# nameofuser1/vad

Measured on NVIDIA B200. Metric: audio_seconds_per_second, higher is better.
Workload: dtype f32

## Files before the change

### include/vadb200.h

```cpp
#ifndef VADB200_H_
#define VADB200_H_

#include <stdint.h>

#ifdef __cplusplus
extern "C" {
#endif

#define VADB200_VERSION 201

#define VADB200_OK 0
#define VADB200_E_INVALID (-1)
#define VADB200_E_UNSUPPORTED (-2)
#define VADB200_E_CUDA (-3)
#define VADB200_E_NOMEM (-4)
#define VADB200_E_STATE (-5)

#define VADB200_MODE_MFCC 0
#define VADB200_MODE_DATASET 1
#define VADB200_MODE_VAD 2

#define VADB200_FEAT_ANALYSER 0
#define VADB200_FEAT_DATASET 1

typedef struct vadb200_handle vadb200_handle;
typedef struct vadb200_plan vadb200_plan;
typedef struct vadb200_bank vadb200_bank;
typedef struct vadb200_trainer vadb200_trainer;

typedef struct vadb200_config {
  int32_t sample_rate;
  int32_t frame_size;
  int32_t frame_step;
  int32_t fft_n;
  int32_t n_filters;
  int32_t n_mfcc;
  double low_hz;
  double high_hz;
  int32_t lifter_l;
  int32_t reserved;
} vadb200_config;

const char* vadb200_last_error(void);
int vadb200_version(void);
void vadb200_default_config(vadb200_config* cfg);

int64_t vadb200_frames_for_length(int64_t n_samples);
int64_t vadb200_outputs_for_length(int64_t n_samples);

int vadb200_create(const vadb200_config* cfg, int device, vadb200_handle** out);
int vadb200_destroy(vadb200_handle* h);

int vadb200_get_filterbank(vadb200_handle* h, double* h_out);

int vadb200_set_ffn_weights(vadb200_handle* h, const float* W1, const float* b1, const float* W2,
                            const float* b2, const float* W3, const float* b3, const float* W4,
                            const float* b4);

int vadb200_set_ffn_impl(vadb200_handle* h, int impl);
int vadb200_get_ffn_impl(vadb200_handle* h);

int vadb200_set_frontend(vadb200_handle* h, float preemph, const float* h_window );
int vadb200_get_frontend(vadb200_handle* h, float* preemph, float* h_window , int* has_window);
int vadb200_set_decision_threshold(vadb200_handle* h, float p_voiced);
float vadb200_get_decision_threshold(vadb200_handle* h);

int vadb200_plan_create(vadb200_handle* h, const int64_t* h_offsets, const int64_t* h_lengths,
                        int64_t n_utt, int mode, vadb200_plan** out);
int vadb200_plan_destroy(vadb200_plan* p);
int64_t vadb200_plan_total_rows(const vadb200_plan* p);
int vadb200_plan_row_offsets(const vadb200_plan* p, int64_t* h_out );
int64_t vadb200_plan_segment_frames(const vadb200_plan* p);
int64_t vadb200_plan_segment_count(const vadb200_plan* p);
int vadb200_set_plan_segment_frames(vadb200_handle* h, int frames);

int vadb200_mfcc_packed(vadb200_plan* p, const int16_t* d_pcm, int64_t pcm_len, float* d_out,
                        void* stream);

int vadb200_vad_packed(vadb200_plan* p, const int16_t* d_pcm, int64_t pcm_len, uint8_t* d_labels,
                       float* d_logits, float* d_feats, int feat_mode, void* stream);

int vadb200_vad_host(vadb200_plan* p, const int16_t* h_pcm, int64_t pcm_len, uint8_t* h_labels,
                     float* h_logits , int feat_mode);
int vadb200_set_host_chunk_samples(vadb200_handle* h, int64_t samples);
int vadb200_mfcc_host(vadb200_plan* p, const int16_t* h_pcm, int64_t pcm_len, float* h_out);

int64_t vadb200_plan_max_speech_segments(const vadb200_plan* p);
int64_t vadb200_plan_speech_workspace_bytes(const vadb200_plan* p);
int vadb200_plan_speech_segments(vadb200_plan* p, const uint8_t* d_labels ,
                                 int min_speech_rows, int min_silence_rows, int pad_rows,
                                 uint8_t* d_smoothed ,
                                 int64_t* d_segments ,
                                 int64_t* d_segment_offsets ,
                                 int64_t* d_speech_offsets ,
                                 void* d_workspace, int64_t workspace_bytes, void* stream);
int vadb200_plan_gather_speech(vadb200_plan* p, const int16_t* d_pcm, int64_t pcm_len,
                               const int64_t* d_segments, const int64_t* d_segment_offsets,
                               const int64_t* d_speech_offsets, int16_t* d_out ,
                               int64_t out_capacity, void* stream);

int vadb200_scale_rows(vadb200_handle* h, float* d_rows, int64_t n_rows, double* h_stats, void* stream);
int vadb200_ingest_pcm(vadb200_handle* h, const void* d_raw, int big_endian, const int64_t* d_src_start,
                       const int64_t* d_dst_start, const int64_t* d_len, int n_seg, int64_t max_len,
                       int16_t* d_dst, void* stream);

int vadb200_spec_frames(vadb200_handle* h, const float* d_frames, int64_t n, int frame_len,
                        float* d_spec , void* stream);
int vadb200_mfcc_frames(vadb200_handle* h, const float* d_frames, int64_t n, int frame_len,
                        float* d_mfcc , void* stream);
int vadb200_mfcc_from_spec(vadb200_handle* h, const float* d_spec , int64_t n,
                           float* d_mfcc , void* stream);

int vadb200_vad_windows(vadb200_handle* h, const float* d_windows, int64_t n, int feat_mode,
                        uint8_t* d_labels , float* d_logits ,
                        float* d_feats , void* stream);
int vadb200_ffn_predict(vadb200_handle* h, const float* d_x, int64_t n, uint8_t* d_labels,
                        float* d_logits , void* stream);

int vadb200_get_deltas(vadb200_handle* h, const float* d_a, const float* d_b, int64_t n,
                       float* d_out, void* stream);
int vadb200_lifter(vadb200_handle* h, const float* d_in, int64_t n_rows, int ncoef, int L,
                   float* d_out, void* stream);

int vadb200_stream_bank_create(vadb200_handle* h, int n_streams, vadb200_bank** out);
int vadb200_stream_bank_destroy(vadb200_bank* b);
int vadb200_stream_bank_reset(vadb200_bank* b, void* stream);
int vadb200_stream_feed(vadb200_bank* b, const int16_t* d_chunks ,
                        uint8_t* d_labels , float* d_logits ,
                        void* stream);

int vadb200_trainer_create(vadb200_handle* h, int64_t max_batch, float lr, float rho, float eps,
                           vadb200_trainer** out);
int vadb200_trainer_destroy(vadb200_trainer* t);
int vadb200_trainer_set_weights(vadb200_trainer* t, const float* W1, const float* b1, const float* W2,
                                const float* b2, const float* W3, const float* b3, const float* W4,
                                const float* b4, int reset_optimizer);
int vadb200_trainer_get_weights(vadb200_trainer* t, float* W1, float* b1, float* W2, float* b2, float* W3,
                                float* b3, float* W4, float* b4);
int vadb200_train_on_batch(vadb200_trainer* t, const float* d_x, const uint8_t* d_y, int64_t n,
                           float* h_loss, void* stream);

int vadb200_synth_pcm(vadb200_handle* h, int16_t* d_out, int64_t n_utt, int64_t utt_samples,
                      int64_t utt_stride, uint32_t seed, int64_t first_utt, void* stream);
int vadb200_fp32_peak(vadb200_handle* h, int variant, int iters, double* tflops_out);
int64_t vadb200_launch_count(void);

#ifdef __cplusplus
}
#endif
#endif
```

### vad_b200/_lib.py

```python
import ctypes as C
import os

HERE = os.path.dirname(os.path.abspath(__file__))
LIB_PATH = os.environ.get("VADB200_LIB") or os.path.join(HERE, "libvadb200.so")


class VadB200Error(RuntimeError):
    def __init__(self, code, msg):
        RuntimeError.__init__(self, "vadb200 error %d: %s" % (code, msg))
        self.code = code


class Config(C.Structure):
    _fields_ = [("sample_rate", C.c_int32), ("frame_size", C.c_int32), ("frame_step", C.c_int32),
                ("fft_n", C.c_int32), ("n_filters", C.c_int32), ("n_mfcc", C.c_int32),
                ("low_hz", C.c_double), ("high_hz", C.c_double), ("lifter_l", C.c_int32),
                ("reserved", C.c_int32)]


_P = C.c_void_p
_I64 = C.c_int64
SIGNATURES = {
    "vadb200_last_error": (C.c_char_p, []),
    "vadb200_version": (C.c_int, []),
    "vadb200_default_config": (None, [C.POINTER(Config)]),
    "vadb200_frames_for_length": (_I64, [_I64]),
    "vadb200_outputs_for_length": (_I64, [_I64]),
    "vadb200_create": (C.c_int, [C.POINTER(Config), C.c_int, C.POINTER(_P)]),
    "vadb200_destroy": (C.c_int, [_P]),
    "vadb200_get_filterbank": (C.c_int, [_P, _P]),
    "vadb200_set_ffn_weights": (C.c_int, [_P] + [_P] * 8),
    "vadb200_set_ffn_impl": (C.c_int, [_P, C.c_int]),
    "vadb200_get_ffn_impl": (C.c_int, [_P]),
    "vadb200_set_frontend": (C.c_int, [_P, C.c_float, _P]),
    "vadb200_get_frontend": (C.c_int, [_P, _P, _P, _P]),
    "vadb200_set_decision_threshold": (C.c_int, [_P, C.c_float]),
    "vadb200_get_decision_threshold": (C.c_float, [_P]),
    "vadb200_plan_create": (C.c_int, [_P, _P, _P, _I64, C.c_int, C.POINTER(_P)]),
    "vadb200_plan_destroy": (C.c_int, [_P]),
    "vadb200_plan_total_rows": (_I64, [_P]),
    "vadb200_plan_row_offsets": (C.c_int, [_P, _P]),
    "vadb200_plan_segment_frames": (_I64, [_P]),
    "vadb200_plan_segment_count": (_I64, [_P]),
    "vadb200_set_plan_segment_frames": (C.c_int, [_P, C.c_int]),
    "vadb200_mfcc_host": (C.c_int, [_P, _P, _I64, _P]),
    "vadb200_plan_max_speech_segments": (_I64, [_P]),
    "vadb200_plan_speech_workspace_bytes": (_I64, [_P]),
    "vadb200_plan_speech_segments": (C.c_int, [_P, _P, C.c_int, C.c_int, C.c_int, _P, _P, _P, _P, _P, _I64, _P]),
    "vadb200_plan_gather_speech": (C.c_int, [_P, _P, _I64, _P, _P, _P, _P, _I64, _P]),
    "vadb200_scale_rows": (C.c_int, [_P, _P, _I64, _P, _P]),
    "vadb200_ingest_pcm": (C.c_int, [_P, _P, C.c_int, _P, _P, _P, C.c_int, _I64, _P, _P]),
    "vadb200_mfcc_packed": (C.c_int, [_P, _P, _I64, _P, _P]),
    "vadb200_vad_packed": (C.c_int, [_P, _P, _I64, _P, _P, _P, C.c_int, _P]),
    "vadb200_vad_host": (C.c_int, [_P, _P, _I64, _P, _P, C.c_int]),
    "vadb200_set_host_chunk_samples": (C.c_int, [_P, _I64]),
    "vadb200_spec_frames": (C.c_int, [_P, _P, _I64, C.c_int, _P, _P]),
    "vadb200_mfcc_frames": (C.c_int, [_P, _P, _I64, C.c_int, _P, _P]),
    "vadb200_mfcc_from_spec": (C.c_int, [_P, _P, _I64, _P, _P]),
    "vadb200_vad_windows": (C.c_int, [_P, _P, _I64, C.c_int, _P, _P, _P, _P]),
    "vadb200_ffn_predict": (C.c_int, [_P, _P, _I64, _P, _P, _P]),
    "vadb200_get_deltas": (C.c_int, [_P, _P, _P, _I64, _P, _P]),
    "vadb200_lifter": (C.c_int, [_P, _P, _I64, C.c_int, C.c_int, _P, _P]),
    "vadb200_stream_bank_create": (C.c_int, [_P, C.c_int, C.POINTER(_P)]),
    "vadb200_stream_bank_destroy": (C.c_int, [_P]),
    "vadb200_stream_bank_reset": (C.c_int, [_P, _P]),
    "vadb200_stream_feed": (C.c_int, [_P, _P, _P, _P, _P]),
    "vadb200_trainer_create": (C.c_int, [_P, _I64, C.c_float, C.c_float, C.c_float, C.POINTER(_P)]),
    "vadb200_trainer_destroy": (C.c_int, [_P]),
    "vadb200_trainer_set_weights": (C.c_int, [_P] + [_P] * 8 + [C.c_int]),
    "vadb200_trainer_get_weights": (C.c_int, [_P] + [_P] * 8),
    "vadb200_train_on_batch": (C.c_int, [_P, _P, _P, _I64, _P, _P]),
    "vadb200_synth_pcm": (C.c_int, [_P, _P, _I64, _I64, _I64, C.c_uint32, _I64, _P]),
    "vadb200_fp32_peak": (C.c_int, [_P, C.c_int, C.c_int, C.POINTER(C.c_double)]),
    "vadb200_launch_count": (_I64, []),
}

_lib = None


def load():
    global _lib
    if _lib is not None:
        return _lib
    if not os.path.isfile(LIB_PATH):
        raise ImportError(
            "vad_b200: %s is missing -- build it with `python -m vad_b200.build` "
            "(nvcc, sm_100a).  There is no CPU fallback." % LIB_PATH)
    lib = C.CDLL(LIB_PATH)
    for name, (res, args) in SIGNATURES.items():
        fn = getattr(lib, name)
        fn.restype = res
        fn.argtypes = args
    _lib = lib
    return lib


def check(rc):
    if rc != 0:
        raise VadB200Error(rc, load().vadb200_last_error().decode("utf-8", "replace"))
```

### vad_b200/csrc/vad_kernels.cuh

```cuda
#pragma once

#include <cuda_runtime.h>

#include "vad_core.cuh"
#include "ffn_tc.cuh"

namespace vadb {

constexpr int kThreads = 256;
constexpr int kWarps = 8;
constexpr int kStepFrames = 32;
constexpr int kRing = 288;
constexpr int kPPitch = 34;
constexpr int kStageSamples = (kStepFrames - 1) * kHop + kFrame;
constexpr int kStagePad = 5376;
constexpr int kBlockSteps = 8;

constexpr int kOffPcm = 0;
constexpr int kOffExch = kOffPcm + 2 * kStagePad * 2;
constexpr int kOffP = kOffExch + kWarps * 2 * kExchFrame * 8;
constexpr int kP2Bytes = (kP2RowsAlloc * kP2Pitch * 4 + 15) & ~15;
constexpr int kOffLogE = kOffP + kP2Bytes;
constexpr int kLogEFloats = kNMel * 32;
constexpr int kOffRing = kOffLogE + 2 * kLogEFloats * 4;
constexpr int kOffTw1 = kOffRing + ((kRingRows * ring_pitch(kRing) * 4 + 15) & ~15);
constexpr int kOffTw2 = kOffTw1 + 256 * 8;
constexpr int kOffBar = kOffTw2 + 128 * 8;
constexpr int kOffSeg = kOffBar + 48;
constexpr int kFusedSmemBytes = kOffSeg + 16;
constexpr int kBlockStepsTc = 4;
static_assert(kTcBlobBytes <= kWarps * 2 * kExchFrame * 8 + kP2Bytes, "weight blob must fit exch + P");
static_assert(kBlockSteps * kStepFrames * kNFeat * 4 + 16 <= kWarps * 2 * kExchFrame * 8 + kP2Bytes,
              "dataset-row staging tile must fit exch + P");
static_assert(2 * (kFusedSmemBytes + 1024) <= 233472, "two CTAs per SM");

struct Segment {
  long long pcm_start;
  long long out_start;
  int n_frames;
  int cont;
};

struct FrontEnd {
  const cf2* win;
  float preemph;
};

#if defined(VADB_DEBUG_HOOKS)
#define VADB_DBG(p) ((p).debug_skip)
#else
#define VADB_DBG(p) 0
#endif

struct FusedParams {
  const int16_t* pcm;
  long long pcm_len;
  const Segment* segs;
  int seg_begin, seg_end;
  int* counter;
  const cf2* tw1;
  const cf2* tw2;
  uint8_t* labels;
  float* logits;
  float* feats;
  float* rows;
  long long row_base;
  int feat_mode;
  const unsigned char* tc_blob;
  long long* dbg_ts;
  int debug_skip;
};

__device__ __forceinline__ uint32_t smem_u32(const void* p) {
  return static_cast<uint32_t>(__cvta_generic_to_shared(p));
}
__device__ __forceinline__ void mbar_init(uint64_t* bar, uint32_t count) {
  asm volatile("mbarrier.init.shared::cta.b64 [%0], %1;" ::"r"(smem_u32(bar)), "r"(count) : "memory");
}
__device__ __forceinline__ void fence_mbar_init() {
  asm volatile("fence.mbarrier_init.release.cluster;" ::: "memory");
}
__device__ __forceinline__ void mbar_arrive_expect_tx(uint64_t* bar, uint32_t bytes) {
  asm volatile("mbarrier.arrive.expect_tx.shared::cta.b64 _, [%0], %1;" ::"r"(smem_u32(bar)), "r"(bytes)
               : "memory");
}
__device__ __forceinline__ void mbar_arrive(uint64_t* bar) {
  asm volatile("mbarrier.arrive.shared::cta.b64 _, [%0];" ::"r"(smem_u32(bar)) : "memory");
}
__device__ __forceinline__ void warp_arrive(uint64_t* bar, int lane) {
  __syncwarp();
  if (lane == 0) mbar_arrive(bar);
}
__device__ __forceinline__ bool mbar_try_wait(uint64_t* bar, uint32_t parity) {
  uint32_t ok;
  asm volatile(
      "{\n\t.reg .pred p;\n\t"
      "mbarrier.try_wait.parity.shared::cta.b64 p, [%1], %2;\n\t"
      "selp.u32 %0, 1, 0, p;\n\t}"
      : "=r"(ok)
      : "r"(smem_u32(bar)), "r"(parity)
      : "memory");
  return ok != 0;
}
__device__ __forceinline__ void mbar_wait(uint64_t* bar, uint32_t parity) {
  while (!mbar_try_wait(bar, parity)) {
  }
}
__device__ __forceinline__ void bulk_g2s(void* dst_smem, const void* src_gmem, uint32_t bytes, uint64_t* bar) {
  asm volatile(
      "cp.async.bulk.shared::cluster.global.mbarrier::complete_tx::bytes [%0], [%1], %2, [%3];" ::"r"(
          smem_u32(dst_smem)),
      "l"(src_gmem), "r"(bytes), "r"(smem_u32(bar))
      : "memory");
}

struct ShflXchg {
  int lane;
  __device__ __forceinline__ float operator()(float mine, int, bool, int partner) const {
    return __shfl_sync(0xffffffffu, mine, (lane & 16) | partner);
  }
  __device__ __forceinline__ f2 operator()(f2 mine, int, bool, int partner) const {
    const int src = (lane & 16) | partner;
    return mk2(__shfl_sync(0xffffffffu, mine.x, src), __shfl_sync(0xffffffffu, mine.y, src));
  }
};

template <int NZ, class LOAD, class PRE, class STORE>
__device__ __forceinline__ void warp_fft_quad(LOAD&& load, f2* ex, const cf2* s_tw1, const cf2* s_tw2, int lane,
                                               PRE&& before_store, STORE&& store) {
  const int t = lane & 15;
  f2 xr[16], xi[16];
  load(t, xr, xi);
  fft_pass1<NZ>(xr, xi, s_tw1, t);
  exch_store_plane(ex, t, xr);
  __syncwarp();
  exch_load_plane(ex, t, xr);
  __syncwarp();
  exch_store_plane(ex, t, xi);
  __syncwarp();
  exch_load_plane(ex, t, xi);
  __syncwarp();
  dft16<16>(xr, xi);
  before_store();
  fft_split_store(xr, xi, t, s_tw2, ShflXchg{lane}, store);
}
struct P2Store {
  static constexpr bool kHasSink = true;
  float* lo_base;
  float* hi_base;
  float* lo0;
  float* mid_ptr;
  __device__ __forceinline__ P2Store(float* P2, int col, int k1) {
    lo_base = P2 + p2_index(k1, col);
    hi_base = P2 + p2_index(256 - k1, col);
    float* sink = P2 + kP2Rows * kP2Pitch + k1 + 2 * (col & 8);
    lo0 = k1 >= kMelFirstBin ? lo_base : sink;
    mid_ptr = k1 == 0 ? P2 + p2_index(128, col) : sink;
  }
  static __device__ __forceinline__ void put(float* q, f2 v) {
    q[0] = v.x;
    q[2] = v.y;
  }
  template <class K> __device__ __forceinline__ void lo(K, f2 v) const {
    constexpr int k2 = K::value;
    if constexpr (k2 == 0) put(lo0, v);
    else put(lo_base + 8 * k2 * kP2Pitch, v);
  }
  template <class K> __device__ __forceinline__ void hi(K, f2 v) const { put(hi_base - 8 * K::value * kP2Pitch, v); }
  __device__ __forceinline__ void mid(f2 v) const { put(mid_ptr, v); }
};

template <int NZ, class LOAD>
__device__ __forceinline__ void warp_fft_pair(LOAD&& load, cf2* ex, const cf2* s_tw1, const cf2* s_tw2,
                                               float* s_P, int fi, int lane) {
  const int t = lane & 15;
  float xr[16], xi[16];
  load(xr, xi);
  fft_pass1<NZ>(xr, xi, s_tw1, t);
  exch_store(ex, t, xr, xi);
  __syncwarp();
  exch_load(ex, t, xr, xi);
  __syncwarp();
  dft16<16>(xr, xi);
  fft_split_store(xr, xi, t, s_tw2, ShflXchg{lane}, [&](int bin, float v) { s_P[bin * kPPitch + fi] = v; });
}

template <int NTHREADS = kThreads, class GEN>
__device__ __forceinline__ void flush_flat(float* dst, int total, int tid, GEN&& gen) {
  if (total <= 0) return;
  const int head = min(total, static_cast<int>((16u - (reinterpret_cast<uintptr_t>(dst) & 15u)) & 15u) >> 2);
  const int nq = (total - head) >> 2;
  for (int q = tid; q < nq; q += NTHREADS) {
    float v[4];
    gen(head + 4 * q, v, 4);
    *reinterpret_cast<float4*>(dst + head + 4 * q) = make_float4(v[0], v[1], v[2], v[3]);
  }
  const int tail0 = head + 4 * nq;
  if (tid < 2) {
    const int j0 = tid == 0 ? 0 : tail0, cnt = tid == 0 ? head : total - tail0;
    if (cnt > 0) {
      float v[4];
      gen(j0, v, cnt);
#pragma unroll
      for (int i = 0; i < 4; ++i)
        if (i < cnt) dst[j0 + i] = v[i];
    }
  }
}

__device__ __forceinline__ void classify_row(const FfnParams& w, const float (&r)[5][kNCep], int feat_mode,
                                             uint8_t* labels, float* logits, float* feats, long long row, float th) {
  float x[kNFeat];
  const bool ok = window_features(r, feat_mode, x);
  float logit[kNCls];
  ffn_forward(w, x, logit);
  uint8_t lab = decide(logit, th);
  if (!ok) {
    logit[0] = logit[1] = logit[2] = NAN;
    lab = 0;
  }
  if (labels) labels[row] = lab;
  if (logits) {
    logits[row * 3 + 0] = logit[0];
    logits[row * 3 + 1] = logit[1];
    logits[row * 3 + 2] = logit[2];
  }
  if (feats) {
#pragma unroll
    for (int i = 0; i < kNFeat; ++i) feats[row * kNFeat + i] = x[i];
  }
}

template <int MODE, int TC> struct FfnArgOf { using type = FfnNone; };
template <> struct FfnArgOf<2, 0> { using type = FfnParams; };
template <> struct FfnArgOf<2, 1> { using type = FfnBias; };
template <> struct FfnArgOf<2, 2> { using type = FfnBias; };

template <bool FE, class A>
__device__ __forceinline__ uint8_t decide_of(const float (&logit)[kNCls], const A& ffn) {
  if constexpr (FE && !std::is_same<A, FfnNone>::value) return decide(logit, ffn.thresh);
  else return decide(logit);
}

constexpr int kStageOffFe = 8;
static_assert(kStageSamples + kStageOffFe <= kStagePad, "front-end stage offset must fit the PCM buffer");

template <int MODE, int TC, bool FE>
__device__ __forceinline__ void fused_body(const FusedParams& p, const typename FfnArgOf<MODE, TC>::type& ffn,
                                           const FrontEnd& fe, const int tid) {
  static_assert(TC == 0 || MODE == 2, "tensor-core FFN only exists in VAD mode");
  constexpr int kBlk = TC ? kBlockStepsTc : kBlockSteps;
  constexpr int kStageOff = FE ? kStageOffFe : 0;
  extern __shared__ __align__(128) unsigned char smem[];
  int16_t* s_pcm = reinterpret_cast<int16_t*>(smem + kOffPcm);
  cf2* s_exch = reinterpret_cast<cf2*>(smem + kOffExch);
  float* s_P = reinterpret_cast<float*>(smem + kOffP);
  float* s_logE = reinterpret_cast<float*>(smem + kOffLogE);
  float* s_ring = reinterpret_cast<float*>(smem + kOffRing);
  cf2* s_tw1 = reinterpret_cast<cf2*>(smem + kOffTw1);
  cf2* s_tw2 = reinterpret_cast<cf2*>(smem + kOffTw2);
  uint64_t* s_bar = reinterpret_cast<uint64_t*>(smem + kOffBar);
  int* s_seg = reinterpret_cast<int*>(smem + kOffSeg);

  const int warp = tid >> 5, lane = tid & 31, h = lane >> 4, t = lane & 15;

  s_tw1[tid] = p.tw1[tid];
  if (tid < 128) s_tw2[tid] = p.tw2[tid];
  uint32_t* s_tmem = reinterpret_cast<uint32_t*>(smem + kOffSeg + 8);
  if (tid == 0) {
    mbar_init(&s_bar[0], 1);
    mbar_init(&s_bar[1], 1);
    mbar_init(&s_bar[2], 1);
    mbar_init(&s_bar[3], 1);
    mbar_init(&s_bar[4], kWarps);
    mbar_init(&s_bar[5], kWarps);
    fence_mbar_init();
  }
  uint32_t tm_base = 0, w_par = 0, mma_par = 0;
  int dbg_n = 0;
  if (TC) {
    if (warp == 0) tmem_alloc(s_tmem, kTmemCols);
    tc_fence_before();
    __syncthreads();
    tc_fence_after();
    tm_base = *s_tmem;
  }

  unsigned gstep = 0;
  Segment seg{};
  const P2Store p2store(s_P, col_of_halfwarp(warp, h), t);
  __syncthreads();
  warp_arrive(&s_bar[4], lane);


  auto issue_load = [&](int step, int buf) {
    const long long start = seg.pcm_start + static_cast<long long>(step) * (kStepFrames * kHop);
    const long long avail = p.pcm_len - start;
    const int nsmp = avail >= kStageSamples ? kStageSamples : (avail > 0 ? static_cast<int>(avail) : 0);
    const int bulk = (nsmp * 2) & ~15;
    int16_t* dst = s_pcm + buf * kStagePad + kStageOff;
    if (tid == 0) {
      mbar_arrive_expect_tx(&s_bar[buf], static_cast<uint32_t>(bulk));
      if (bulk) bulk_g2s(dst, p.pcm + start, static_cast<uint32_t>(bulk), &s_bar[buf]);
    }
    const int tail0 = bulk >> 1;
    if (tid < nsmp - tail0) dst[tail0 + tid] = p.pcm[start + tail0 + tid];
    if (FE && tid == 31) dst[-1] = (step > 0 || seg.cont) ? p.pcm[start - 1] : int16_t(0);
  };

  for (;;) {
    __syncthreads();
    if (tid == 0) *s_seg = p.seg_begin + atomicAdd(p.counter, 1);
    __syncthreads();
    const int si = *s_seg;
    if (si >= p.seg_end) break;
    seg = p.segs[si];
    const int n = seg.n_frames;
    const int nsteps = (n + kStepFrames - 1) / kStepFrames;
    int out_done = (MODE == 0) ? 0 : 2;
    bool dct_pending = false;
    if (nsteps > 0 && warp == 0) issue_load(0, gstep & 1);
    __syncthreads();

    for (int s = 0; s < nsteps; ++s, ++gstep) {
      const int buf = gstep & 1;
      if (s + 1 < nsteps && warp == 0) issue_load(s + 1, buf ^ 1);
      mbar_wait(&s_bar[buf], (gstep >> 1) & 1);

      const uint32_t par = gstep & 1;
      auto dct_step = [&](int sd) {
        if (!(VADB_DBG(p) & 4)) {
          const float* le = s_logE + (sd & 1) * kLogEFloats + lane;
          const int col = (sd * kStepFrames + slot_of_col(lane)) % kRing;
          if (warp < 3) {
            float ra, rb, rc, rd;
            dct_coef4<32>(le, 2 * warp, ra, rb, rc, rd);
            *reinterpret_cast<float2*>(s_ring + ring_idx(4 * warp, col, kRing)) = make_float2(ra, rb);
            *reinterpret_cast<float2*>(s_ring + ring_idx(4 * warp + 2, col, kRing)) = make_float2(rc, rd);
          } else if (warp == 3) {
            float ra, rb;
            dct_coef2<32>(le, 6, ra, rb);
            s_ring[ring_idx(12, col, kRing)] = ra;
          }
        }
      };

      const uint32_t* stage32 = reinterpret_cast<const uint32_t*>(s_pcm + buf * kStagePad + kStageOff);
      if (!(VADB_DBG(p) & 1)) {
        f2* ex = reinterpret_cast<f2*>(s_exch) + (warp * 2 + h) * kExchFrame;
        const uint32_t* w32a = stage32 + (warp * 4 + h) * (kHop / 2);
        warp_fft_quad<13>(
            [&](int tt, f2 (&xr)[16], f2 (&xi)[16]) {
              if constexpr (FE) fft_load_pcm2_fe(w32a, kHop, tt, fe.preemph, fe.win, xr, xi);
              else fft_load_pcm2(w32a, kHop, tt, xr, xi);
            },
            ex, s_tw1, s_tw2, lane, [&] { mbar_wait(&s_bar[4], par); }, p2store);
      } else {
        mbar_wait(&s_bar[4], par);
      }
      warp_arrive(&s_bar[5], lane);

      if (dct_pending) dct_step(s - 1);
      mbar_wait(&s_bar[5], par);

      if (!(VADB_DBG(p) & 2))
        mel2_run_dispatch<kP2Pitch, 32>(warp, s_P + 2 * lane, s_logE + (s & 1) * kLogEFloats + lane);
      warp_arrive(&s_bar[4], lane);
      const int computed = min((s + 1) * kStepFrames, n);
      const bool block_now = (((s + 1) % kBlk) == 0 || s == nsteps - 1) && !(VADB_DBG(p) & 8);
      const bool tc_now = TC && block_now && (computed - 2 - out_done) > 0;
      dct_pending = !block_now;

      if (block_now) {
        if (tc_now) asm volatile("fence.proxy.async.shared::cta;" ::: "memory");
        __syncthreads();
        if (tc_now && tid == 0 && !(VADB_DBG(p) & 16)) {
          constexpr uint32_t blob_bytes = TC == 2 ? kTc16BlobBytes : kTcBlobBytes;
          mbar_arrive_expect_tx(&s_bar[2], blob_bytes);
          bulk_g2s(smem + kOffExch, p.tc_blob, blob_bytes, &s_bar[2]);
        }
        dct_step(s);
      }

      if (block_now) {
        __syncthreads();
        if (MODE == 0) {
          float* dst = p.rows + (seg.out_start - p.row_base + out_done) * kNCep;
          const int first = out_done;
          flush_flat(dst, (computed - out_done) * kNCep, tid, [&](int j, float (&v)[4], int cnt) {
            int fr = j / kNCep, cf = j - fr * kNCep;
#pragma unroll
            for (int i = 0; i < 4; ++i) {
              if (i < cnt) v[i] = s_ring[ring_idx(cf, (first + fr) % kRing, kRing)];
              if (++cf == kNCep) { cf = 0; ++fr; }
            }
          });
          out_done = computed;
        } else if (MODE == 1) {
          const int n_valid = computed - 2 - out_done;
          if (n_valid > 0) {
            float* dst = p.rows + (seg.out_start - p.row_base + (out_done - 2)) * kNFeat;
            float* stage = reinterpret_cast<float*>(smem + kOffExch) + ((reinterpret_cast<uintptr_t>(dst) & 15u) >> 2);
            if (tid < n_valid) {
              float xa[24], xb[24];
              window_features_pairs<0, 4, kRing, 24>(s_ring, out_done + tid, 1, xa);
              window_features_pairs<4, 7, kRing, 24>(s_ring, out_done + tid, 1, xb);
              float* row = stage + tid * kNFeat;
#pragma unroll
              for (int g = 0; g < 3; ++g) {
#pragma unroll
                for (int k = 0; k < 8; ++k) row[g * kNCep + k] = xa[6 * (k >> 1) + 2 * g + (k & 1)];
#pragma unroll
                for (int k = 0; k < 5; ++k) row[g * kNCep + 8 + k] = xb[6 * (k >> 1) + 2 * g + (k & 1)];
              }
            }
            __syncthreads();
            flush_flat(dst, n_valid * kNFeat, tid, [&](int j, float (&v)[4], int cnt) {
              if (cnt == 4) {
                const float4 q = *reinterpret_cast<const float4*>(stage + j);
                v[0] = q.x; v[1] = q.y; v[2] = q.z; v[3] = q.w;
              } else {
#pragma unroll
                for (int i = 0; i < 4; ++i)
                  if (i < cnt) v[i] = stage[j + i];
              }
            });
            __syncthreads();
          }
          out_done = max(out_done, computed - 2);
        } else if (!TC) {
          const int c = out_done + tid;
          if (c <= computed - 3) {
            float r[5][kNCep];
#pragma unroll
            for (int d = 0; d < 5; ++d) {
              const int col = (c - 2 + d) % kRing;
#pragma unroll
              for (int k = 0; k < kNCep; ++k) r[d][k] = s_ring[ring_idx(k, col, kRing)];
            }
            if constexpr (MODE == 2 && TC == 0)
              classify_row(ffn, r, p.feat_mode, p.labels, p.logits, p.feats, seg.out_start - p.row_base + (c - 2),
                           FE ? ffn.thresh : 0.0f);
          }
          out_done = max(out_done, computed - 2);
        } else {
          const int n_valid = computed - 2 - out_done;
          if (n_valid > 0) {
            unsigned char* wdst = smem + kOffExch;
            {
              const int fr = tid & 127, hidx = tid >> 7;
              long long* ts = nullptr;
#if defined(VADB_DEBUG_HOOKS)
              if (p.dbg_ts && blockIdx.x == 0 && tid == 0 && dbg_n < 64) ts = p.dbg_ts + 16 * dbg_n;
#endif
              if (ts) ts[0] = clock64();
              const bool valid = fr < n_valid;
              const int c = out_done + (valid ? fr : 0);
              const uint32_t tl = tm_base + (static_cast<uint32_t>(32 * (warp & 3)) << 16);
              float xl[24], logit[kNCls];
              bool ok_half = true;
              if (VADB_DBG(p) & 64) {
#pragma unroll
                for (int i = 0; i < 24; ++i) xl[i] = 0.5f;
              } else {
                ok_half = (hidx == 0) ? window_features_pairs<0, 4, kRing, 24>(s_ring, c, p.feat_mode, xl)
                                      : window_features_pairs<4, 7, kRing, 24>(s_ring, c, p.feat_mode, xl);
              }
              s_logE[tid] = ok_half ? 1.0f : 0.0f;
              if (ts) ts[1] = clock64();
              if constexpr (TC == 2) tc16_store_a1_half(tl, hidx, xl);
              else tc_store_a1_half(tl, hidx, xl);
              if (p.feats && valid) {
                const long long row = seg.out_start - p.row_base + (c - 2);
                const int k0 = hidx ? 8 : 0, nk = hidx ? 5 : 8;
#pragma unroll
                for (int k = 0; k < 8; ++k)
#pragma unroll
                  for (int g = 0; g < 3; ++g)
                    if (k < nk) p.feats[row * kNFeat + g * kNCep + k0 + k] = xl[6 * (k >> 1) + 2 * g + (k & 1)];
              }
              if (!(VADB_DBG(p) & 16)) mbar_wait(&s_bar[2], w_par);
              if (ts) ts[2] = clock64();
              if constexpr (TC == 1)
                mma_par = ffn_tc_tile<2>(ffn, logit, tm_base, warp & 3, hidx, tid == 0, smem_u32(wdst), &s_bar[3], mma_par,
                                         ts, VADB_DBG(p));
              if constexpr (TC == 2)
                mma_par = ffn_tc16_tile<2>(ffn, logit, tm_base, warp & 3, hidx, tid == 0, smem_u32(wdst), &s_bar[3], mma_par);
              ++dbg_n;
              if (valid && hidx == 0) {
                const bool ok = s_logE[fr] != 0.0f && s_logE[128 + fr] != 0.0f;
                uint8_t lab = decide_of<FE>(logit, ffn);
                if (!ok) {
                  logit[0] = logit[1] = logit[2] = NAN;
                  lab = 0;
                }
                const long long row = seg.out_start - p.row_base + (c - 2);
                p.labels[row] = lab;
                if (p.logits) {
                  p.logits[row * 3 + 0] = logit[0];
                  p.logits[row * 3 + 1] = logit[1];
                  p.logits[row * 3 + 2] = logit[2];
                }
              }
            }
            if (!(VADB_DBG(p) & 16)) w_par ^= 1u;
            __syncthreads();
          }
          out_done = max(out_done, computed - 2);
        }
      }
    }
  }
  if (TC) {
    tc_fence_before();
    __syncthreads();
    if (warp == 0) tmem_dealloc(tm_base, kTmemCols);
  }
  if (tid == 0) {
    __threadfence();
    if (atomicAdd(p.counter + 1, 1) == static_cast<int>(gridDim.x) - 1) {
      p.counter[0] = 0;
      p.counter[1] = 0;
      __threadfence();
    }
  }
}

template <int MODE, int TC>
__global__ void __launch_bounds__(kThreads, 2) fused_kernel(const __grid_constant__ FusedParams p,
                                                            const __grid_constant__ typename FfnArgOf<MODE, TC>::type ffn) {
  fused_body<MODE, TC, false>(p, ffn, FrontEnd{nullptr, 0.0f}, threadIdx.x);
}
template <int MODE, int TC>
__global__ void __launch_bounds__(kThreads, 2) fused_fe_kernel(const __grid_constant__ FusedParams p,
                                                               const __grid_constant__ typename FfnArgOf<MODE, TC>::type ffn,
                                                               const __grid_constant__ FrontEnd fe) {
  fused_body<MODE, TC, true>(p, ffn, fe, threadIdx.x);
}

constexpr int kFfnTcSmemBytes = kTcBlobBytes + 64;
template <int KIND>
__global__ void __launch_bounds__(128) ffn_tc_rows_kernel(const float* x, long long n, const unsigned char* blob16,
                                                          const unsigned char* blob32, uint8_t* labels, float* logits,
                                                          const __grid_constant__ FfnBias fb) {
  extern __shared__ __align__(128) unsigned char smem[];
  uint64_t* bars = reinterpret_cast<uint64_t*>(smem + kTcBlobBytes);
  uint32_t* s_tmem = reinterpret_cast<uint32_t*>(smem + kTcBlobBytes + 32);
  const int tid = threadIdx.x, warp = tid >> 5;
  if (tid == 0) {
    mbar_init(&bars[0], 1);
    mbar_init(&bars[1], 1);
    fence_mbar_init();
  }
  if (warp == 0) tmem_alloc(s_tmem, kTmemCols);
  tc_fence_before();
  __syncthreads();
  tc_fence_after();
  const uint32_t tm_base = *s_tmem;
  if (KIND == 1 && tid == 0) {
    mbar_arrive_expect_tx(&bars[0], kTcBlobBytes);
    bulk_g2s(smem, blob32, kTcBlobBytes, &bars[0]);
  }
  const long long i = static_cast<long long>(blockIdx.x) * 128 + tid;
  const long long src = i < n ? i : n - 1;
  float v[kNFeat], logit[kNCls];
  bool ok = true, wide = false;
#pragma unroll
  for (int k = 0; k < kNFeat; ++k) {
    v[k] = x[src * kNFeat + k];
    ok = ok && (fabsf(v[k]) <= 3.0e38f);
    if constexpr (KIND == 2)
      wide = wide || fabsf(v[k]) > (k < kNCep ? kFeatBoundZ : k < 2 * kNCep ? kFeatBoundD1 : kFeatBoundD2);
  }
  bool fp16 = false;
  if constexpr (KIND == 2) {
    fp16 = !__syncthreads_or(wide);
    if (tid == 0) {
      const uint32_t bytes = fp16 ? kTc16BlobBytes : kTcBlobBytes;
      mbar_arrive_expect_tx(&bars[0], bytes);
      bulk_g2s(smem, fp16 ? blob16 : blob32, bytes, &bars[0]);
    }
  }
  mbar_wait(&bars[0], 0);
  {
    const uint32_t tl = tm_base + (static_cast<uint32_t>(32 * warp) << 16);
    float h0[24], h1[24];
#pragma unroll
    for (int i = 0; i < 24; ++i) h0[i] = h1[i] = 0.0f;
#pragma unroll
    for (int f = 0; f < kNFeat; ++f) {
      const int col = tc_feat_col(f);
      if (col < 24) h0[col] = v[f];
      else h1[col - 24] = v[f];
    }
    if (fp16) {
      tc16_store_a1_half(tl, 0, h0);
      tc16_store_a1_half(tl, 1, h1);
    } else {
      tc_store_a1_half(tl, 0, h0);
      tc_store_a1_half(tl, 1, h1);
    }
  }
  if (fp16) ffn_tc16_tile<1>(fb, logit, tm_base, warp, 0, tid == 0, smem_u32(smem), &bars[1], 0);
  else ffn_tc_tile<1>(fb, logit, tm_base, warp, 0, tid == 0, smem_u32(smem), &bars[1], 0);
  if (i < n) {
    uint8_t lab = decide(logit, fb.thresh);
    if (!ok) {
      logit[0] = logit[1] = logit[2] = NAN;
      lab = 0;
    }
    if (labels) labels[i] = lab;
    if (logits) {
      logits[i * 3 + 0] = logit[0];
      logits[i * 3 + 1] = logit[1];
      logits[i * 3 + 2] = logit[2];
    }
  }
  tc_fence_before();
  __syncthreads();
  if (warp == 0) tmem_dealloc(tm_base, kTmemCols);
}

#if defined(VADB_DEBUG_HOOKS)
constexpr int kExpSmemBytes = 2 * kStagePad * 2 + kWarps * 2 * kExchFrame * 8 + 384 * 8 + 64;
template <int MINB>
__global__ void __launch_bounds__(kThreads, MINB) exp_fft_kernel(const FusedParams p, float* sink) {
  extern __shared__ __align__(128) unsigned char smem[];
  int16_t* s_pcm = reinterpret_cast<int16_t*>(smem);
  cf2* s_exch = reinterpret_cast<cf2*>(smem + 2 * kStagePad * 2);
  cf2* s_tw1 = reinterpret_cast<cf2*>(smem + 2 * kStagePad * 2 + kWarps * 2 * kExchFrame * 8);
  cf2* s_tw2 = s_tw1 + 256;
  uint64_t* s_bar = reinterpret_cast<uint64_t*>(s_tw2 + 128);
  int* s_seg = reinterpret_cast<int*>(s_bar + 4);
  const int tid = threadIdx.x, warp = tid >> 5, lane = tid & 31, h = lane >> 4, t = lane & 15;
  s_tw1[tid] = p.tw1[tid];
  if (tid < 128) s_tw2[tid] = p.tw2[tid];
  if (tid == 0) {
    mbar_init(&s_bar[0], 1);
    mbar_init(&s_bar[1], 1);
    fence_mbar_init();
  }
  unsigned gstep = 0;
  float acc = 0.0f;
  Segment seg;
  auto issue_load = [&](int step, int buf) {
    const long long start = seg.pcm_start + static_cast<long long>(step) * (kStepFrames * kHop);
    const long long avail = p.pcm_len - start;
    const int nsmp = avail >= kStageSamples ? kStageSamples : (avail > 0 ? static_cast<int>(avail) : 0);
    const int bulk = (nsmp * 2) & ~15;
    if (tid == 0) {
      mbar_arrive_expect_tx(&s_bar[buf], static_cast<uint32_t>(bulk));
      if (bulk) bulk_g2s(s_pcm + buf * kStagePad, p.pcm + start, static_cast<uint32_t>(bulk), &s_bar[buf]);
    }
  };
  for (;;) {
    __syncthreads();
    if (tid == 0) *s_seg = p.seg_begin + atomicAdd(p.counter, 1);
    __syncthreads();
    const int si = *s_seg;
    if (si >= p.seg_end) break;
    seg = p.segs[si];
    const int nsteps = (seg.n_frames + kStepFrames - 1) / kStepFrames;
    issue_load(0, gstep & 1);
    __syncthreads();
    for (int s = 0; s < nsteps; ++s, ++gstep) {
      const int buf = gstep & 1;
      if (s + 1 < nsteps) issue_load(s + 1, buf ^ 1);
      mbar_wait(&s_bar[buf], (gstep >> 1) & 1);
      const uint32_t* stage32 = reinterpret_cast<const uint32_t*>(s_pcm + buf * kStagePad);
      cf2* ex = s_exch + (warp * 2 + h) * kExchFrame;
#pragma unroll 1
      for (int r = 0; r < 2; ++r) {
        const int fi = warp * 4 + r * 2 + h;
        const uint32_t* w32 = stage32 + fi * (kHop / 2);
        float xr[16], xi[16];
        fft_load_pcm(w32, t, xr, xi);
        fft_pass1<13>(xr, xi, s_tw1, t);
        exch_store(ex, t, xr, xi);
        __syncwarp();
        exch_load(ex, t, xr, xi);
        __syncwarp();
        dft16<16>(xr, xi);
        fft_split_store(xr, xi, t, s_tw2, ShflXchg{lane}, [&](int bin, float v) { acc = fmaf(v, 1e-12f * bin, acc); });
      }
      __syncthreads();
    }
  }
  if (acc == 123.456f) sink[0] = acc;
}
#endif

constexpr int kFramesSmemBytes = kWarps * 2 * kExchFrame * 8 + kBins * kPPitch * 4 + kNMel * 32 * 4 + 384 * 8;

__global__ void __launch_bounds__(kThreads) frames_kernel(const float* frames, long long n, int frame_len, int what,
                                                         float* out, const cf2* tw1, const cf2* tw2, FrontEnd fe) {
  extern __shared__ __align__(128) unsigned char smem[];
  cf2* s_exch = reinterpret_cast<cf2*>(smem);
  float* s_P = reinterpret_cast<float*>(smem + kWarps * 2 * kExchFrame * 8);
  float* s_logE = s_P + kBins * kPPitch;
  cf2* s_tw1 = reinterpret_cast<cf2*>(s_logE + kNMel * 32);
  cf2* s_tw2 = s_tw1 + 256;
  const int tid = threadIdx.x, warp = tid >> 5, lane = tid & 31, h = lane >> 4, t = lane & 15;
  s_tw1[tid] = tw1[tid];
  if (tid < 128) s_tw2[tid] = tw2[tid];
  __syncthreads();
  const long long f0 = static_cast<long long>(blockIdx.x) * kStepFrames;
  cf2* ex = s_exch + (warp * 2 + h) * kExchFrame;
#pragma unroll 1
  for (int r = 0; r < 2; ++r) {
    const int fi = warp * 4 + r * 2 + h;
    const long long f = min(f0 + fi, n - 1);
    const float* fr = frames + f * frame_len;
    warp_fft_pair<16>(
        [&](float (&xr)[16], float (&xi)[16]) {
          if (fe.win) fft_load_f32_fe(fr, frame_len, t, fe.preemph, fe.win, xr, xi);
          else fft_load_f32(fr, frame_len, t, xr, xi);
        },
        ex, s_tw1, s_tw2, s_P, fi, lane);
  }
  __syncthreads();
  if (what == 0) {
    for (int j = tid; j < kStepFrames * kBins; j += kThreads) {
      const int fi = j >> 8, k = j & 255;
      if (f0 + fi < n) out[(f0 + fi) * kBins + k] = s_P[k * kPPitch + fi] * 9.5367431640625e-07f;
    }
    return;
  }
  mel_group_dispatch<kPPitch, 32>(warp, s_P + lane, s_logE + lane);
  __syncthreads();
  if (f0 + lane < n) {
    out[(f0 + lane) * kNCep + warp] = dct_coef<32>(s_logE + lane, warp);
    if (warp + 8 < kNCep) out[(f0 + lane) * kNCep + warp + 8] = dct_coef<32>(s_logE + lane, warp + 8);
  }
}

__global__ void __launch_bounds__(kThreads) spec_to_mfcc_kernel(const float* spec, long long n, float* out) {
  __shared__ float s_P[kBins * kPPitch];
  __shared__ float s_logE[kNMel * 32];
  const int tid = threadIdx.x, warp = tid >> 5, lane = tid & 31;
  const long long f0 = static_cast<long long>(blockIdx.x) * kStepFrames;
  for (int j = tid; j < kStepFrames * kBins; j += kThreads) {
    const int fi = j >> 8, k = j & 255;
    const long long f = min(f0 + fi, n - 1);
    s_P[k * kPPitch + fi] = spec[f * kBins + k] * 1048576.0f;
  }
  __syncthreads();
  mel_group_dispatch<kPPitch, 32>(warp, s_P + lane, s_logE + lane);
  __syncthreads();
  if (f0 + lane < n) {
    out[(f0 + lane) * kNCep + warp] = dct_coef<32>(s_logE + lane, warp);
    if (warp + 8 < kNCep) out[(f0 + lane) * kNCep + warp + 8] = dct_coef<32>(s_logE + lane, warp + 8);
  }
}

__global__ void __launch_bounds__(128) windows_kernel(const float* win, long long n, int feat_mode, uint8_t* labels,
                                                      float* logits, float* feats, const __grid_constant__ FfnParams w) {
  const long long i = static_cast<long long>(blockIdx.x) * blockDim.x + threadIdx.x;
  if (i >= n) return;
  float r[5][kNCep];
#pragma unroll
  for (int d = 0; d < 5; ++d)
#pragma unroll
    for (int k = 0; k < kNCep; ++k) r[d][k] = win[(i * 5 + d) * kNCep + k];
  classify_row(w, r, feat_mode, labels, logits, feats, i, w.thresh);
}

__global__ void __launch_bounds__(128) ffn_rows_kernel(const float* x, long long n, uint8_t* labels, float* logits,
                                                       const __grid_constant__ FfnParams w) {
  const long long i = static_cast<long long>(blockIdx.x) * blockDim.x + threadIdx.x;
  if (i >= n) return;
  float v[kNFeat];
  bool ok = true;
#pragma unroll
  for (int k = 0; k < kNFeat; ++k) {
    v[k] = x[i * kNFeat + k];
    ok = ok && (fabsf(v[k]) <= 3.0e38f);
  }
  float logit[kNCls];
  ffn_forward(w, v, logit);
  uint8_t lab = decide(logit, w.thresh);
  if (!ok) {
    logit[0] = logit[1] = logit[2] = NAN;
    lab = 0;
  }
  if (labels) labels[i] = lab;
  if (logits) {
    logits[i * 3 + 0] = logit[0];
    logits[i * 3 + 1] = logit[1];
    logits[i * 3 + 2] = logit[2];
  }
}

__global__ void elementwise_kernel(int op, const float* a, const float* b, long long n, int ncoef, int L, float* out) {
  const long long i = static_cast<long long>(blockIdx.x) * blockDim.x + threadIdx.x;
  if (i >= n) return;
  if (op == 0) {
    out[i] = a[i] - b[i];
  } else {
    const int k = static_cast<int>(i % ncoef);
    const float lift = (L > 0) ? 1.0f + (0.5f * L) * sinpif(static_cast<float>(k) / static_cast<float>(L)) : 1.0f;
    out[i] = lift * a[i];
  }
}

struct BankParams {
  int n_streams;
  int16_t* hist;
  float* ring;
  int* fed;
  const int16_t* chunks;
  uint8_t* labels;
  float* logits;
  const cf2* tw1;
  const cf2* tw2;
  int feat_mode;
  int16_t* prev;
  FrontEnd fe;
};
constexpr int kStreamFramePitch = 480;
constexpr int kStreamPBytes = kP2Bytes > (kNFeat + kH1 + kH2 + kH3 + kNCep) * 32 * 4
                                  ? kP2Bytes : (kNFeat + kH1 + kH2 + kH3 + kNCep) * 32 * 4;
constexpr int kStreamRowsOff = 16;
constexpr int kStreamSmemBytes = kStreamRowsOff + kStepFrames * kStreamFramePitch * 2 + kWarps * 2 * kExchFrame * 8 +
                                 kStreamPBytes + kNMel * 32 * 4 + 384 * 8;

__global__ void __launch_bounds__(kThreads) stream_feed_kernel(const BankParams p, const __grid_constant__ FfnParams w) {
  extern __shared__ __align__(128) unsigned char smem[];
  int16_t* s_fr = reinterpret_cast<int16_t*>(smem + kStreamRowsOff);
  cf2* s_exch = reinterpret_cast<cf2*>(smem + kStreamRowsOff + kStepFrames * kStreamFramePitch * 2);
  float* s_P = reinterpret_cast<float*>(reinterpret_cast<unsigned char*>(s_exch) + kWarps * 2 * kExchFrame * 8);
  float* s_logE = reinterpret_cast<float*>(reinterpret_cast<unsigned char*>(s_P) + kStreamPBytes);
  cf2* s_tw1 = reinterpret_cast<cf2*>(s_logE + kNMel * 32);
  cf2* s_tw2 = s_tw1 + 256;
  float* s_x = s_P;
  float* s_h1 = s_x + kNFeat * 32;
  float* s_h2 = s_h1 + kH1 * 32;
  float* s_h3 = s_h2 + kH2 * 32;
  int* s_ok = reinterpret_cast<int*>(s_h3 + kH3 * 32);
  const int tid = threadIdx.x, warp = tid >> 5, lane = tid & 31, h = lane >> 4;
  const int s0 = blockIdx.x * kStepFrames;
  s_tw1[tid] = p.tw1[tid];
  if (tid < 128) s_tw2[tid] = p.tw2[tid];
  for (int j = tid; j < kStepFrames * 240; j += kThreads) {
    const int fi = j / 240, wd = j - fi * 240;
    const int st = min(s0 + fi, p.n_streams - 1);
    const uint32_t v = (wd < 160) ? reinterpret_cast<const uint32_t*>(p.hist + static_cast<long long>(st) * 320)[wd]
                                  : reinterpret_cast<const uint32_t*>(p.chunks + static_cast<long long>(st) * 160)[wd - 160];
    reinterpret_cast<uint32_t*>(s_fr + fi * kStreamFramePitch)[wd] = v;
  }
  __syncthreads();
  for (int j = tid; j < kStepFrames * 160; j += kThreads) {
    const int fi = j / 160, wd = j - fi * 160;
    const int st = s0 + fi;
    if (st < p.n_streams)
      reinterpret_cast<uint32_t*>(p.hist + static_cast<long long>(st) * 320)[wd] =
          reinterpret_cast<const uint32_t*>(s_fr + fi * kStreamFramePitch)[80 + wd];
  }
  if (p.fe.win) {
    __syncthreads();
    if (tid < kStepFrames) {
      int16_t* row = s_fr + tid * kStreamFramePitch;
      const int st = min(s0 + tid, p.n_streams - 1);
      row[-1] = p.prev[st];
      if (s0 + tid < p.n_streams) p.prev[st] = row[159];
    }
    __syncthreads();
  }
  {
    f2* ex = reinterpret_cast<f2*>(s_exch) + (warp * 2 + h) * kExchFrame;
    const uint32_t* w32 = reinterpret_cast<const uint32_t*>(s_fr + (warp * 4 + h) * kStreamFramePitch);
    warp_fft_quad<13>(
        [&](int t, f2 (&xr)[16], f2 (&xi)[16]) {
          if (p.fe.win) fft_load_pcm2_fe(w32, kStreamFramePitch, t, p.fe.preemph, p.fe.win, xr, xi);
          else fft_load_pcm2(w32, kStreamFramePitch, t, xr, xi);
        },
        ex, s_tw1, s_tw2, lane, [] {}, P2Store(s_P, col_of_halfwarp(warp, h), lane & 15));
  }
  __syncthreads();
  mel2_run_dispatch<kP2Pitch, 32>(warp, s_P + 2 * lane, s_logE + lane);
  __syncthreads();
  const int slot = slot_of_col(lane);
  const int st = s0 + slot;
  const bool live = st < p.n_streams;
  const long long ns = p.n_streams;
  const int fed = live ? p.fed[st] : 0;
  const int frame = fed - 2;
#pragma unroll
  for (int rep = 0; rep < 2; ++rep) {
    const int k = warp + 8 * rep;
    if (k < kNCep) {
      const float cnew = dct_coef<32>(s_logE + lane, k);
      float r[5] = {0.f, 0.f, 0.f, 0.f, 0.f};
      if (live && frame >= 0) {
#pragma unroll
        for (int d = 0; d < 5; ++d) r[d] = p.ring[(d * kNCep + k) * ns + st];
#pragma unroll
        for (int d = 0; d < 4; ++d) p.ring[(d * kNCep + k) * ns + st] = r[d + 1];
        p.ring[(4 * kNCep + k) * ns + st] = cnew;
      }
      float z = r[2];
      bool ok = true;
      if (p.feat_mode == 0) {
        const float mu = ((((r[0] + r[1]) + r[2]) + r[3]) + r[4]) * 0.2f;
        const float d0 = r[0] - mu, d1 = r[1] - mu, d2 = r[2] - mu, d3 = r[3] - mu, d4 = r[4] - mu;
        const float var = fmaf(d4, d4, fmaf(d3, d3, fmaf(d2, d2, fmaf(d1, d1, d0 * d0)))) * 0.2f;
        const bool alleq = (r[0] == r[1]) && (r[1] == r[2]) && (r[2] == r[3]) && (r[3] == r[4]);
        z = alleq ? NAN : d2 * vadb_rsqrt(var);
        ok = fabsf(z) <= 3.0e38f;
      }
      s_x[k * 32 + slot] = z;
      s_x[(kNCep + k) * 32 + slot] = r[3] - r[1];
      s_x[(2 * kNCep + k) * 32 + slot] = (r[4] - z) - (z - r[0]);
      s_ok[k * 32 + slot] = ok ? 1 : 0;
    }
  }
  __syncthreads();
  {
    float acc[8];
#pragma unroll
    for (int j = 0; j < 8; ++j) acc[j] = w.b1[8 * warp + j];
#pragma unroll 3
    for (int i = 0; i < kNFeat; ++i) {
      const float xv = s_x[i * 32 + lane];
#pragma unroll
      for (int j = 0; j < 8; ++j) acc[j] = fmaf(xv, w.W1[i * kH1 + 8 * warp + j], acc[j]);
    }
#pragma unroll
    for (int j = 0; j < 8; ++j) s_h1[(8 * warp + j) * 32 + lane] = fmaxf(acc[j], 0.0f);
  }
  __syncthreads();
  {
    float acc[4];
#pragma unroll
    for (int j = 0; j < 4; ++j) acc[j] = w.b2[4 * warp + j];
#pragma unroll 4
    for (int i = 0; i < kH1; ++i) {
      const float a = s_h1[i * 32 + lane];
#pragma unroll
      for (int j = 0; j < 4; ++j) acc[j] = fmaf(a, w.W2[i * kH2 + 4 * warp + j], acc[j]);
    }
#pragma unroll
    for (int j = 0; j < 4; ++j) s_h2[(4 * warp + j) * 32 + lane] = fmaxf(acc[j], 0.0f);
  }
  __syncthreads();
  {
    float acc[2];
#pragma unroll
    for (int j = 0; j < 2; ++j) acc[j] = w.b3[2 * warp + j];
#pragma unroll 4
    for (int i = 0; i < kH2; ++i) {
      const float a = s_h2[i * 32 + lane];
#pragma unroll
      for (int j = 0; j < 2; ++j) acc[j] = fmaf(a, w.W3[i * kH3 + 2 * warp + j], acc[j]);
    }
#pragma unroll
    for (int j = 0; j < 2; ++j) s_h3[(2 * warp + j) * 32 + lane] = fmaxf(acc[j], 0.0f);
  }
  __syncthreads();
  if (warp == 0) {
    const int stl = s0 + lane;
    if (stl < p.n_streams) {
      const int fedl = p.fed[stl];
      uint8_t lab = 255;
      float lg[3] = {NAN, NAN, NAN};
      if (fedl - 2 >= 5) {
        float acc[kNCls];
#pragma unroll
        for (int o = 0; o < kNCls; ++o) acc[o] = w.b4[o];
#pragma unroll
        for (int i = 0; i < kH3; ++i) {
          const float a = s_h3[i * 32 + lane];
#pragma unroll
          for (int o = 0; o < kNCls; ++o) acc[o] = fmaf(a, w.W4[i * kNCls + o], acc[o]);
        }
        bool ok = true;
#pragma unroll
        for (int k = 0; k < kNCep; ++k) ok = ok && (s_ok[k * 32 + lane] != 0);
        lab = decide(acc, w.thresh);
        if (ok) {
          lg[0] = acc[0]; lg[1] = acc[1]; lg[2] = acc[2];
        } else {
          lab = 0;
        }
      }
      p.fed[stl] = fedl + 1;
      p.labels[stl] = lab;
      if (p.logits) {
        p.logits[stl * 3 + 0] = lg[0];
        p.logits[stl * 3 + 1] = lg[1];
        p.logits[stl * 3 + 2] = lg[2];
      }
    }
  }
}

__device__ __forceinline__ double warp_sum(double v) {
#pragma unroll
  for (int o = 16; o > 0; o >>= 1) v += __shfl_down_sync(0xffffffffu, v, o);
  return v;
}
__global__ void __launch_bounds__(256) scale_rows_kernel(float* rows, long long n_rows, int pass, double* acc) {
  const long long total = n_rows * kNFeat;
  const double cnt = static_cast<double>(n_rows) * kNCep;
  double m0 = 0.0, m1 = 0.0, m2 = 0.0, i0 = 0.0, i1 = 0.0, i2 = 0.0;
  if (pass >= 1) {
    m0 = acc[0] / cnt; m1 = acc[1] / cnt; m2 = acc[2] / cnt;
  }
  if (pass == 2) {
    i0 = 1.0 / sqrt(acc[3] / cnt); i1 = 1.0 / sqrt(acc[4] / cnt); i2 = 1.0 / sqrt(acc[5] / cnt);
  }
  double p0 = 0.0, p1 = 0.0, p2 = 0.0;
  const long long stride = static_cast<long long>(gridDim.x) * blockDim.x;
  for (long long j = static_cast<long long>(blockIdx.x) * blockDim.x + threadIdx.x; j < total; j += stride) {
    const int col = static_cast<int>(j % kNFeat);
    const int g = col / kNCep;
    const double v = static_cast<double>(rows[j]);
    const double mean = g == 0 ? m0 : g == 1 ? m1 : m2;
    if (pass == 0) {
      p0 += g == 0 ? v : 0.0; p1 += g == 1 ? v : 0.0; p2 += g == 2 ? v : 0.0;
    } else if (pass == 1) {
      const double d = v - mean, dd = d * d;
      p0 += g == 0 ? dd : 0.0; p1 += g == 1 ? dd : 0.0; p2 += g == 2 ? dd : 0.0;
    } else {
      rows[j] = static_cast<float>((v - mean) * (g == 0 ? i0 : g == 1 ? i1 : i2));
    }
  }
  if (pass == 2) return;
  __shared__ double s_part[3][8];
  const int warp = threadIdx.x >> 5, lane = threadIdx.x & 31;
  {
    const double w0 = warp_sum(p0), w1 = warp_sum(p1), w2 = warp_sum(p2);
    if (lane == 0) { s_part[0][warp] = w0; s_part[1][warp] = w1; s_part[2][warp] = w2; }
  }
  __syncthreads();
  if (threadIdx.x < 3) {
    double t = 0.0;
    for (int w = 0; w < 8; ++w) t += s_part[threadIdx.x][w];
    atomicAdd(acc + 3 * pass + threadIdx.x, t);
  }
}

__global__ void __launch_bounds__(256) ingest_kernel(const uint8_t* raw, int big_endian, const long long* src,
                                                     const long long* dst_off, const long long* len, int16_t* dst) {
  const int seg = blockIdx.y;
  const long long n = len[seg];
  const uint16_t* in = reinterpret_cast<const uint16_t*>(raw) + src[seg];
  int16_t* out = dst + dst_off[seg];
  const long long stride = static_cast<long long>(gridDim.x) * blockDim.x;
  for (long long k = static_cast<long long>(blockIdx.x) * blockDim.x + threadIdx.x; k < n; k += stride) {
    uint16_t v = in[k];
    if (big_endian) v = static_cast<uint16_t>((v << 8) | (v >> 8));
    out[k] = static_cast<int16_t>(v);
  }
}

__device__ __forceinline__ uint32_t mix32(uint32_t x) {
  x ^= x >> 16; x *= 0x7FEB352Du; x ^= x >> 15; x *= 0x846CA68Bu; x ^= x >> 16;
  return x;
}
__global__ void synth_kernel(int16_t* out, long long n_utt, long long utt_samples, long long utt_stride, uint32_t seed,
                             long long first_utt) {
  const long long total = n_utt * utt_samples;
  for (long long g = static_cast<long long>(blockIdx.x) * blockDim.x + threadIdx.x; g < total;
       g += static_cast<long long>(gridDim.x) * blockDim.x) {
    const long long u = g / utt_samples;
    const uint32_t i = static_cast<uint32_t>(g - u * utt_samples);
    const uint32_t key = mix32(mix32(seed ^ 0x9E3779B9u) + static_cast<uint32_t>(first_utt + u));
    const uint32_t a = mix32(key + i);
    const uint32_t b = mix32(a ^ 0x85EBCA6Bu);
    const int s = static_cast<int>((a & 0xFFFFu) + (a >> 16) + (b & 0xFFFFu) + (b >> 16)) - 131070;
    const uint32_t gh = mix32((key ^ 0x5BD1E995u) + (i >> 11));
    const int gain = (gh & 0x1000u) ? static_cast<int>(1500u + (gh & 0xFFFu)) : static_cast<int>(40u + (gh & 0x7Fu));
    out[u * utt_stride + i] = static_cast<int16_t>((s * gain) >> 16);
  }
}

template <int VARIANT>
__global__ void __launch_bounds__(256) fp32_peak_kernel(float* sink, int iters, float m, float a) {
  float acc[16];
#pragma unroll
  for (int i = 0; i < 16; ++i) acc[i] = static_cast<float>(threadIdx.x + i);
  for (int it = 0; it < iters; ++it) {
#pragma unroll
    for (int rep = 0; rep < 8; ++rep) {
#pragma unroll
      for (int i = 0; i < 16; ++i) {
        if (VARIANT == 0) acc[i] = fmaf(acc[i], m, a);
        else acc[i] = fmaf(acc[i], c_tab.melw[rep * 16 + i], a);
      }
    }
  }
  float s = 0.0f;
#pragma unroll
  for (int i = 0; i < 16; ++i) s += acc[i];
  if (s == 123.456f) sink[0] = s;
}
template <int VARIANT>
__global__ void __launch_bounds__(256) fp32x2_peak_kernel(float* sink, int iters, float m, float a) {
  float2 acc[16];
#pragma unroll
  for (int i = 0; i < 16; ++i) acc[i] = make_float2(static_cast<float>(threadIdx.x + i), static_cast<float>(i));
  const float2 m2 = make_float2(m, m + 1e-7f), a2 = make_float2(a, a);
  for (int it = 0; it < iters; ++it) {
#pragma unroll
    for (int rep = 0; rep < 8; ++rep) {
#pragma unroll
      for (int i = 0; i < 16; ++i) {
        if (VARIANT == 2) acc[i] = __ffma2_rn(acc[i], m2, a2);
        else acc[i] = __ffma2_rn(acc[i], make_float2(1.0000001f, 1.0000001f), a2);
      }
    }
  }
  float s = 0.0f;
#pragma unroll
  for (int i = 0; i < 16; ++i) s += acc[i].x + acc[i].y;
  if (s == 123.456f) sink[0] = s;
}
template <int NS>
__global__ void __launch_bounds__(256) fp32mix_peak_kernel(float* sink, int iters, float m, float a) {
  float2 acc2[8];
  float acc[NS > 0 ? NS : 1];
#pragma unroll
  for (int i = 0; i < 8; ++i) acc2[i] = make_float2(static_cast<float>(threadIdx.x + i), static_cast<float>(i));
#pragma unroll
  for (int i = 0; i < NS; ++i) acc[i] = static_cast<float>(threadIdx.x - i);
  const float2 a2 = make_float2(a, a);
  for (int it = 0; it < iters; ++it) {
#pragma unroll
    for (int rep = 0; rep < 8; ++rep) {
#pragma unroll
      for (int i = 0; i < 8; ++i) {
        acc2[i] = __ffma2_rn(acc2[i], make_float2(1.0000001f, 1.0000001f), a2);
        if (i < NS) acc[i] = fmaf(acc[i], m, a);
      }
    }
  }
  float s = 0.0f;
#pragma unroll
  for (int i = 0; i < 8; ++i) s += acc2[i].x + acc2[i].y;
#pragma unroll
  for (int i = 0; i < NS; ++i) s += acc[i];
  if (s == 123.456f) sink[0] = s;
}

}
```

### vad_b200/csrc/vadb200.cu

```cuda
#include "../../include/vadb200.h"

#include <cuda_runtime.h>

#include <algorithm>
#include <atomic>
#include <cmath>
#include <cstdio>
#include <cstdlib>
#include <cstring>
#include <mutex>
#include <new>
#include <string>
#include <vector>

#include "vad_host_tables.h"
#include "vad_kernels.cuh"
#include "ffn_train.cuh"
#include "vad_segments.cuh"

using namespace vadb;

namespace {

thread_local std::string g_err;
std::atomic<long long> g_launches{0};
std::atomic<unsigned long long> g_next_id{1};
std::mutex g_tab_mu;
bool g_tab_loaded[64] = {false};

int fail(int code, const std::string& msg) {
  g_err = msg;
  return code;
}
int cuda_fail(cudaError_t e, const char* what) {
  g_err = std::string(what) + ": " + cudaGetErrorString(e);
  return VADB200_E_CUDA;
}
#define CU(expr)                                     \
  do {                                               \
    cudaError_t e__ = (expr);                        \
    if (e__ != cudaSuccess) return cuda_fail(e__, #expr); \
  } while (0)

long long* g_dbg_ts = nullptr;
constexpr int kNumSmFallback = 148;
constexpr int kPlanCounters = 16;
constexpr int kHostBufs = 3;
constexpr int kWinPairs = kFftN / 2;

}

struct vadb200_handle {
  int device = 0;
  unsigned long long id = 0;
  unsigned version = 1;
  MfccConfig cfg;
  std::vector<double> fb;
  MelDctTables tab;
  FfnParams par;
  FfnBias bias;
  int plan_seg_frames = 0;
  bool have_ffn = false;
  cf2* d_tw = nullptr;
  int num_sms = kNumSmFallback;
  bool attr_set = false;
  long long host_chunk_samples = 32ll << 20;
  cudaStream_t s_in = nullptr, s_run = nullptr, s_out = nullptr;
  cudaEvent_t ev_in[kHostBufs] = {}, ev_done[kHostBufs] = {}, ev_out[kHostBufs] = {};
  int16_t* d_stage[kHostBufs] = {};
  uint8_t* d_lab[kHostBufs] = {};
  float* d_lgt[kHostBufs] = {};
  float* d_rows[kHostBufs] = {};
  long long stage_cap = 0, lab_cap = 0, lgt_cap = 0, rows_cap = 0;
  float* d_sink = nullptr;
  unsigned char* d_tc_blob = nullptr;
  unsigned char* d_tc16_blob = nullptr;
  bool tc16_ok = false;
  int ffn_impl = 2;
  float preemph = 0.0f;
  bool has_window = false;
  float window[kFrame] = {};
  cf2* d_win = nullptr;
};

struct vadb200_plan {
  vadb200_handle* h = nullptr;
  int mode = 0;
  long long n_utt = 0;
  std::vector<long long> offsets, lengths, row_off, utt_seg;
  std::vector<Segment> segs;
  Segment* d_segs = nullptr;
  int* d_counter = nullptr;
  std::atomic<unsigned> launch_seq{0};
  long long total_rows = 0;
  long long seg_frames = 0;
  std::vector<SpeechTile> tiles;
  std::vector<int> utt_tile;
  long long max_speech_segs = 0;
  long long* d_row_off = nullptr;
  long long* d_pcm_off = nullptr;
  SpeechTile* d_tiles = nullptr;
  int* d_utt_tile = nullptr;
};

struct vadb200_trainer {
  vadb200_handle* h = nullptr;
  long long max_batch = 0;
  float lr = 1.0f, rho = 0.95f, eps = 1e-8f;
  float* d_state = nullptr;
  float* d_partial = nullptr;
  float* d_loss = nullptr;
  long long steps = 0;
};

struct vadb200_bank {
  vadb200_handle* h = nullptr;
  int n = 0;
  int16_t* d_hist = nullptr;
  float* d_ring = nullptr;
  int* d_fed = nullptr;
  int16_t* d_prev = nullptr;
};

namespace {

int ensure_tables(vadb200_handle* h) {
  if (h->device >= 64) return fail(VADB200_E_INVALID, "device index >= 64");
  std::lock_guard<std::mutex> lk(g_tab_mu);
  if (g_tab_loaded[h->device]) return 0;
  CU(cudaMemcpyToSymbol(c_tab, &h->tab, sizeof(MelDctTables), 0, cudaMemcpyHostToDevice));
  CU(cudaDeviceSynchronize());
  g_tab_loaded[h->device] = true;
  return 0;
}

int ensure_attrs(vadb200_handle* h) {
  if (h->attr_set) return 0;
  CU(cudaFuncSetAttribute(fused_kernel<0, 0>, cudaFuncAttributeMaxDynamicSharedMemorySize, kFusedSmemBytes));
  CU(cudaFuncSetAttribute(fused_kernel<1, 0>, cudaFuncAttributeMaxDynamicSharedMemorySize, kFusedSmemBytes));
  CU(cudaFuncSetAttribute(fused_kernel<2, 0>, cudaFuncAttributeMaxDynamicSharedMemorySize, kFusedSmemBytes));
  CU(cudaFuncSetAttribute(fused_kernel<2, 1>, cudaFuncAttributeMaxDynamicSharedMemorySize, kFusedSmemBytes));
  CU(cudaFuncSetAttribute(fused_kernel<2, 2>, cudaFuncAttributeMaxDynamicSharedMemorySize, kFusedSmemBytes));
  CU(cudaFuncSetAttribute(fused_fe_kernel<0, 0>, cudaFuncAttributeMaxDynamicSharedMemorySize, kFusedSmemBytes));
  CU(cudaFuncSetAttribute(fused_fe_kernel<1, 0>, cudaFuncAttributeMaxDynamicSharedMemorySize, kFusedSmemBytes));
  CU(cudaFuncSetAttribute(fused_fe_kernel<2, 0>, cudaFuncAttributeMaxDynamicSharedMemorySize, kFusedSmemBytes));
  CU(cudaFuncSetAttribute(fused_fe_kernel<2, 1>, cudaFuncAttributeMaxDynamicSharedMemorySize, kFusedSmemBytes));
  CU(cudaFuncSetAttribute(fused_fe_kernel<2, 2>, cudaFuncAttributeMaxDynamicSharedMemorySize, kFusedSmemBytes));
  CU(cudaFuncSetAttribute(ffn_tc_rows_kernel<1>, cudaFuncAttributeMaxDynamicSharedMemorySize, kFfnTcSmemBytes));
  CU(cudaFuncSetAttribute(ffn_tc_rows_kernel<2>, cudaFuncAttributeMaxDynamicSharedMemorySize, kFfnTcSmemBytes));
  CU(cudaFuncSetAttribute(frames_kernel, cudaFuncAttributeMaxDynamicSharedMemorySize, kFramesSmemBytes));
  CU(cudaFuncSetAttribute(stream_feed_kernel, cudaFuncAttributeMaxDynamicSharedMemorySize, kStreamSmemBytes));
  h->attr_set = true;
  return 0;
}

bool frontend_on(const vadb200_handle* h) { return h->preemph != 0.0f || h->has_window; }
FrontEnd frontend_of(const vadb200_handle* h) { return FrontEnd{h->d_win, h->preemph}; }

int launch_fused(vadb200_plan* p, FusedParams fp, int n_segs, cudaStream_t st) {
  vadb200_handle* h = p->h;
  if (n_segs <= 0) return 0;
  int rc = ensure_attrs(h);
  if (rc) return rc;
  rc = ensure_tables(h);
  if (rc) return rc;
  fp.counter = p->d_counter + 2 * (p->launch_seq.fetch_add(1) % kPlanCounters);
#if defined(VADB_DEBUG_HOOKS)
  const char* gps = std::getenv("VADB200_CTAS_PER_SM");
  const int per_sm = gps ? std::max(1, std::atoi(gps)) : 2;
#else
  const int per_sm = 2;
#endif
  const int grid = std::min(n_segs, per_sm * h->num_sms);
  const bool fe = frontend_on(h) || (p->mode == VADB200_MODE_VAD && h->par.thresh > 0.0f);
  const FrontEnd fea = frontend_of(h);
  if (fe) {
    switch (p->mode) {
      case VADB200_MODE_MFCC: fused_fe_kernel<0, 0><<<grid, kThreads, kFusedSmemBytes, st>>>(fp, FfnNone{0}, fea); break;
      case VADB200_MODE_DATASET: fused_fe_kernel<1, 0><<<grid, kThreads, kFusedSmemBytes, st>>>(fp, FfnNone{0}, fea); break;
      default:
        if (h->ffn_impl == 2 && h->tc16_ok) {
          fp.tc_blob = h->d_tc16_blob;
          fused_fe_kernel<2, 2><<<grid, kThreads, kFusedSmemBytes, st>>>(fp, h->bias, fea);
        } else if (h->ffn_impl >= 1) {
          fused_fe_kernel<2, 1><<<grid, kThreads, kFusedSmemBytes, st>>>(fp, h->bias, fea);
        } else {
          fused_fe_kernel<2, 0><<<grid, kThreads, kFusedSmemBytes, st>>>(fp, h->par, fea);
        }
        break;
    }
    g_launches.fetch_add(1);
    CU(cudaGetLastError());
    return 0;
  }
  switch (p->mode) {
    case VADB200_MODE_MFCC: fused_kernel<0, 0><<<grid, kThreads, kFusedSmemBytes, st>>>(fp, FfnNone{0}); break;
    case VADB200_MODE_DATASET: fused_kernel<1, 0><<<grid, kThreads, kFusedSmemBytes, st>>>(fp, FfnNone{0}); break;
    default:
      if (h->ffn_impl == 2 && h->tc16_ok) {
        fp.tc_blob = h->d_tc16_blob;
        fused_kernel<2, 2><<<grid, kThreads, kFusedSmemBytes, st>>>(fp, h->bias);
      } else if (h->ffn_impl >= 1) {
        fused_kernel<2, 1><<<grid, kThreads, kFusedSmemBytes, st>>>(fp, h->bias);
      } else {
        fused_kernel<2, 0><<<grid, kThreads, kFusedSmemBytes, st>>>(fp, h->par);
      }
      break;
  }
  g_launches.fetch_add(1);
  CU(cudaGetLastError());
  return 0;
}

FusedParams base_params(vadb200_plan* p) {
  FusedParams fp;
  std::memset(&fp, 0, sizeof(fp));
  fp.segs = p->d_segs;
  fp.counter = p->d_counter;
  fp.tw1 = p->h->d_tw;
  fp.tw2 = p->h->d_tw + 256;
  fp.tc_blob = p->h->d_tc_blob;
#if defined(VADB_DEBUG_HOOKS)
  const char* dbg = std::getenv("VADB200_DEBUG_SKIP");
  fp.debug_skip = dbg ? std::atoi(dbg) : 0;
  fp.dbg_ts = g_dbg_ts;
#else
  fp.debug_skip = 0;
  fp.dbg_ts = nullptr;
#endif
  return fp;
}

}

extern "C" {

const char* vadb200_last_error(void) { return g_err.c_str(); }
int vadb200_version(void) { return VADB200_VERSION; }
int64_t vadb200_launch_count(void) { return g_launches.load(); }
int vadb200_debug_timestamps(long long* d_buf) { g_dbg_ts = d_buf; return 0; }

void vadb200_default_config(vadb200_config* c) {
  if (!c) return;
  c->sample_rate = 16000; c->frame_size = 400; c->frame_step = 160; c->fft_n = 512;
  c->n_filters = 26; c->n_mfcc = 13; c->low_hz = 300.0; c->high_hz = 8000.0; c->lifter_l = 22;
  c->reserved = 0;
}

int64_t vadb200_frames_for_length(int64_t n) { return frames_for_length(n); }
int64_t vadb200_outputs_for_length(int64_t n) { return outputs_for_length(n); }

int vadb200_create(const vadb200_config* c, int device, vadb200_handle** out) {
  if (!out) return fail(VADB200_E_INVALID, "out is null");
  *out = nullptr;
  vadb200_config dc;
  if (!c) {
    vadb200_default_config(&dc);
    c = &dc;
  }
  MfccConfig cfg;
  cfg.sample_rate = c->sample_rate; cfg.frame_size = c->frame_size; cfg.frame_step = c->frame_step;
  cfg.fft_n = c->fft_n; cfg.n_filters = c->n_filters; cfg.n_mfcc = c->n_mfcc;
  cfg.low_hz = c->low_hz; cfg.high_hz = c->high_hz; cfg.lifter_l = c->lifter_l;
  if (!is_reference_config(cfg))
    return fail(VADB200_E_UNSUPPORTED,
                "only the reference configuration (16 kHz, 400/160, n_fft 512, 26 filters 300-8000 Hz, 13 "
                "cepstra, lifter 22; config.py:20-27) is compiled in");
  int ndev = 0;
  CU(cudaGetDeviceCount(&ndev));
  if (device < 0 || device >= ndev) return fail(VADB200_E_INVALID, "no such CUDA device");
  CU(cudaSetDevice(device));
  cudaDeviceProp prop;
  CU(cudaGetDeviceProperties(&prop, device));
  if (prop.major < 10)
    return fail(VADB200_E_UNSUPPORTED, "kernels are built for sm_100a (B200) only");
  vadb200_handle* h = new (std::nothrow) vadb200_handle();
  if (!h) return fail(VADB200_E_NOMEM, "host allocation failed");
  h->device = device;
  h->id = g_next_id.fetch_add(1);
  h->cfg = cfg;
  h->num_sms = prop.multiProcessorCount > 0 ? prop.multiProcessorCount : kNumSmFallback;
  h->fb = mel_filterbank(cfg);
  std::fill(h->window, h->window + kFrame, 1.0f);
  std::memset(&h->par, 0, sizeof(FfnParams));
  std::memset(&h->bias, 0, sizeof(FfnBias));
  std::memset(&h->tab, 0, sizeof(MelDctTables));
  std::string why;
  if (!pack_mel_weights(h->fb.data(), h->tab.melw, &why)) {
    delete h;
    return fail(VADB200_E_UNSUPPORTED, why);
  }
  folded_dct(cfg, h->tab.dct);
  pack_mel_pairs(h->fb.data(), h->tab.melw2);
  pack_dct_pairs(h->tab.dct, h->tab.dctp);
  cf2 tw[384];
  fft_twiddles(tw, tw + 256);
  cudaError_t e = cudaMalloc(&h->d_tw, sizeof(tw));
  if (e == cudaSuccess) e = cudaMemcpy(h->d_tw, tw, sizeof(tw), cudaMemcpyHostToDevice);
  if (e == cudaSuccess) e = cudaMalloc(&h->d_sink, 256);
  if (e == cudaSuccess) e = cudaMalloc(&h->d_tc_blob, kTcBlobBytes);
  if (e == cudaSuccess) e = cudaMalloc(&h->d_tc16_blob, kTc16BlobBytes);
  if (e == cudaSuccess) e = cudaMalloc(&h->d_win, kWinPairs * sizeof(cf2));
  if (e == cudaSuccess) {
    std::vector<cf2> ones(kWinPairs, cf2{1.0f, 1.0f});
    e = cudaMemcpy(h->d_win, ones.data(), kWinPairs * sizeof(cf2), cudaMemcpyHostToDevice);
  }
  if (e != cudaSuccess) {
    cudaFree(h->d_tw);
    cudaFree(h->d_sink);
    cudaFree(h->d_tc_blob);
    cudaFree(h->d_tc16_blob);
    cudaFree(h->d_win);
    delete h;
    return cuda_fail(e, "vadb200_create");
  }
  int rc = ensure_attrs(h);
  if (!rc) rc = ensure_tables(h);
  if (rc) {
    const std::string keep = g_err;
    vadb200_destroy(h);
    g_err = keep;
    return rc;
  }
  *out = h;
  return 0;
}

int vadb200_destroy(vadb200_handle* h) {
  if (!h) return 0;
  cudaSetDevice(h->device);
  for (int i = 0; i < kHostBufs; ++i) {
    cudaFree(h->d_stage[i]); cudaFree(h->d_lab[i]); cudaFree(h->d_lgt[i]); cudaFree(h->d_rows[i]);
    if (h->ev_in[i]) cudaEventDestroy(h->ev_in[i]);
    if (h->ev_done[i]) cudaEventDestroy(h->ev_done[i]);
    if (h->ev_out[i]) cudaEventDestroy(h->ev_out[i]);
  }
  if (h->s_in) cudaStreamDestroy(h->s_in);
  if (h->s_run) cudaStreamDestroy(h->s_run);
  if (h->s_out) cudaStreamDestroy(h->s_out);
  cudaFree(h->d_tw);
  cudaFree(h->d_sink);
  cudaFree(h->d_tc_blob);
  cudaFree(h->d_tc16_blob);
  cudaFree(h->d_win);
  delete h;
  return 0;
}

int vadb200_get_filterbank(vadb200_handle* h, double* out) {
  if (!h || !out) return fail(VADB200_E_INVALID, "null argument");
  std::memcpy(out, h->fb.data(), h->fb.size() * sizeof(double));
  return 0;
}

int vadb200_set_ffn_weights(vadb200_handle* h, const float* W1, const float* b1, const float* W2, const float* b2,
                            const float* W3, const float* b3, const float* W4, const float* b4) {
  if (!h || !W1 || !b1 || !W2 || !b2 || !W3 || !b3 || !W4 || !b4) return fail(VADB200_E_INVALID, "null argument");
  std::memcpy(h->par.W1, W1, sizeof(h->par.W1)); std::memcpy(h->par.b1, b1, sizeof(h->par.b1));
  std::memcpy(h->par.W2, W2, sizeof(h->par.W2)); std::memcpy(h->par.b2, b2, sizeof(h->par.b2));
  std::memcpy(h->par.W3, W3, sizeof(h->par.W3)); std::memcpy(h->par.b3, b3, sizeof(h->par.b3));
  std::memcpy(h->par.W4, W4, sizeof(h->par.W4)); std::memcpy(h->par.b4, b4, sizeof(h->par.b4));
  std::memcpy(h->bias.b1, b1, sizeof(h->bias.b1)); std::memcpy(h->bias.b2, b2, sizeof(h->bias.b2));
  std::memcpy(h->bias.b3, b3, sizeof(h->bias.b3)); std::memcpy(h->bias.b4, b4, sizeof(h->bias.b4));
  h->have_ffn = true;
  h->version = (h->version + 1) & 0xFFFFF;
  std::vector<unsigned char> blob(kTcBlobBytes);
  tc_pack_weights(h->par, blob.data());
  CU(cudaSetDevice(h->device));
  CU(cudaDeviceSynchronize());
  CU(cudaMemcpy(h->d_tc_blob, blob.data(), kTcBlobBytes, cudaMemcpyHostToDevice));
  std::vector<unsigned char> blob16(kTc16BlobBytes);
  h->tc16_ok = tc16_pack_weights(h->par, blob16.data(), h->bias);
  if (h->tc16_ok) CU(cudaMemcpy(h->d_tc16_blob, blob16.data(), kTc16BlobBytes, cudaMemcpyHostToDevice));
  return 0;
}

int vadb200_set_ffn_impl(vadb200_handle* h, int impl) {
  if (!h || impl < 0 || impl > 2)
    return fail(VADB200_E_INVALID, "impl must be 0 (fp32), 1 (tcgen05 tf32 hi/lo) or 2 (tcgen05 fp16 hi/lo)");
  h->ffn_impl = impl;
  return 0;
}
int vadb200_get_ffn_impl(vadb200_handle* h) { return h ? h->ffn_impl : -1; }

int vadb200_set_frontend(vadb200_handle* h, float preemph, const float* h_window) {
  if (!h) return fail(VADB200_E_INVALID, "handle is null");
  if (!(preemph >= 0.0f && preemph <= 1.0f)) return fail(VADB200_E_INVALID, "pre-emphasis must be in [0, 1]");
  if (h_window)
    for (int i = 0; i < kFrame; ++i)
      if (!std::isfinite(h_window[i])) return fail(VADB200_E_INVALID, "window weights must be finite");
  std::vector<cf2> pairs(kWinPairs, cf2{1.0f, 1.0f});
  if (h_window)
    for (int m = 0; m < kFrame / 2; ++m) pairs[m] = cf2{h_window[2 * m], h_window[2 * m + 1]};
  CU(cudaSetDevice(h->device));
  CU(cudaDeviceSynchronize());
  CU(cudaMemcpy(h->d_win, pairs.data(), kWinPairs * sizeof(cf2), cudaMemcpyHostToDevice));
  h->preemph = preemph;
  h->has_window = h_window != nullptr;
  if (h_window) std::memcpy(h->window, h_window, sizeof(h->window));
  else std::fill(h->window, h->window + kFrame, 1.0f);
  return 0;
}

int vadb200_get_frontend(vadb200_handle* h, float* preemph, float* h_window, int* has_window) {
  if (!h) return fail(VADB200_E_INVALID, "handle is null");
  if (preemph) *preemph = h->preemph;
  if (has_window) *has_window = h->has_window ? 1 : 0;
  if (h_window) std::memcpy(h_window, h->window, sizeof(h->window));
  return 0;
}

int vadb200_set_decision_threshold(vadb200_handle* h, float p_voiced) {
  if (!h) return fail(VADB200_E_INVALID, "handle is null");
  if (!(p_voiced < 1.0f)) return fail(VADB200_E_INVALID, "threshold must be < 1 (<= 0: argmax)");
  const float th = p_voiced > 0.0f ? p_voiced : 0.0f;
  h->par.thresh = th;
  h->bias.thresh = th;
  return 0;
}

float vadb200_get_decision_threshold(vadb200_handle* h) { return h ? h->par.thresh : NAN; }

int vadb200_set_host_chunk_samples(vadb200_handle* h, int64_t samples) {
  if (!h || samples < 4096) return fail(VADB200_E_INVALID, "chunk must be >= 4096 samples");
  h->host_chunk_samples = samples & ~7ll;
  return 0;
}

int vadb200_plan_create(vadb200_handle* h, const int64_t* offs, const int64_t* lens, int64_t n_utt, int mode,
                        vadb200_plan** out) {
  if (!h || !out || n_utt < 0 || (n_utt > 0 && (!offs || !lens))) return fail(VADB200_E_INVALID, "null / negative argument");
  if (mode < 0 || mode > 2) return fail(VADB200_E_INVALID, "unknown mode");
  *out = nullptr;
  vadb200_plan* p = new (std::nothrow) vadb200_plan();
  if (!p) return fail(VADB200_E_NOMEM, "host allocation failed");
  p->h = h; p->mode = mode; p->n_utt = n_utt;
  p->offsets.assign(offs, offs + n_utt);
  p->lengths.assign(lens, lens + n_utt);
  p->row_off.resize(n_utt + 1);
  p->utt_seg.resize(n_utt + 1);
  long long rows = 0, prev_end = 0;
  for (long long u = 0; u < n_utt; ++u) {
    if (offs[u] < 0 || (offs[u] & 7) || lens[u] < 0 || offs[u] < prev_end) {
      delete p;
      return fail(VADB200_E_INVALID, "utterance offsets must be ascending, non-overlapping multiples of 8 samples");
    }
    prev_end = offs[u] + lens[u];
    p->row_off[u] = rows;
    rows += (mode == VADB200_MODE_MFCC) ? frames_for_length(lens[u]) : outputs_for_length(lens[u]);
  }
  p->row_off[n_utt] = rows;
  p->total_rows = rows;
  const int halo = (mode == VADB200_MODE_MFCC) ? 0 : 4;
  long long seg_frames = h->plan_seg_frames;
  if (seg_frames <= 0) {
    const long long want = rows / (16ll * 2 * h->num_sms) + halo;
    seg_frames = want <= 64 ? 64 : std::min<long long>(2048, ((want + 127) / 128) * 128);
  }
  p->seg_frames = seg_frames;
  const long long seg_rows = seg_frames - halo;
  for (long long u = 0; u < n_utt; ++u) {
    p->utt_seg[u] = static_cast<long long>(p->segs.size());
    const long long r = p->row_off[u + 1] - p->row_off[u];
    for (long long o = 0; o < r; o += seg_rows) {
      Segment s;
      s.pcm_start = offs[u] + kHop * o;
      s.out_start = p->row_off[u] + o;
      s.n_frames = static_cast<int>(std::min(seg_rows, r - o) + halo);
      s.cont = o > 0 ? 1 : 0;
      p->segs.push_back(s);
    }
  }
  p->utt_seg[n_utt] = static_cast<long long>(p->segs.size());
  if (p->segs.size() > 0x7fffffffull) {
    delete p;
    return fail(VADB200_E_INVALID, "too many segments");
  }
  cudaError_t e = cudaSetDevice(h->device);
  if (e == cudaSuccess) e = cudaMalloc(&p->d_counter, 2 * kPlanCounters * sizeof(int));
  if (e == cudaSuccess) e = cudaMemset(p->d_counter, 0, 2 * kPlanCounters * sizeof(int));
  if (e == cudaSuccess && !p->segs.empty()) {
    e = cudaMalloc(&p->d_segs, p->segs.size() * sizeof(Segment));
    if (e == cudaSuccess)
      e = cudaMemcpy(p->d_segs, p->segs.data(), p->segs.size() * sizeof(Segment), cudaMemcpyHostToDevice);
  }
  if (mode != VADB200_MODE_MFCC) {
    p->utt_tile.resize(n_utt + 1);
    for (long long u = 0; u < n_utt; ++u) {
      p->utt_tile[u] = static_cast<int>(p->tiles.size());
      const long long r = p->row_off[u + 1] - p->row_off[u];
      p->max_speech_segs += (r + 1) / 2;
      for (long long o = 0; o < r; o += kSpeechTile)
        p->tiles.push_back(SpeechTile{p->row_off[u] + o, static_cast<int>(std::min<long long>(kSpeechTile, r - o)),
                                      static_cast<int>(u)});
    }
    p->utt_tile[n_utt] = static_cast<int>(p->tiles.size());
    if (e == cudaSuccess) e = cudaMalloc(&p->d_row_off, (n_utt + 1) * sizeof(long long));
    if (e == cudaSuccess)
      e = cudaMemcpy(p->d_row_off, p->row_off.data(), (n_utt + 1) * sizeof(long long), cudaMemcpyHostToDevice);
    if (e == cudaSuccess) e = cudaMalloc(&p->d_utt_tile, (n_utt + 1) * sizeof(int));
    if (e == cudaSuccess)
      e = cudaMemcpy(p->d_utt_tile, p->utt_tile.data(), (n_utt + 1) * sizeof(int), cudaMemcpyHostToDevice);
    if (e == cudaSuccess && n_utt > 0) {
      e = cudaMalloc(&p->d_pcm_off, n_utt * sizeof(long long));
      if (e == cudaSuccess)
        e = cudaMemcpy(p->d_pcm_off, p->offsets.data(), n_utt * sizeof(long long), cudaMemcpyHostToDevice);
    }
    if (e == cudaSuccess && !p->tiles.empty()) {
      e = cudaMalloc(&p->d_tiles, p->tiles.size() * sizeof(SpeechTile));
      if (e == cudaSuccess)
        e = cudaMemcpy(p->d_tiles, p->tiles.data(), p->tiles.size() * sizeof(SpeechTile), cudaMemcpyHostToDevice);
    }
  }
  if (e != cudaSuccess) {
    cudaFree(p->d_counter); cudaFree(p->d_segs);
    cudaFree(p->d_row_off); cudaFree(p->d_pcm_off); cudaFree(p->d_tiles); cudaFree(p->d_utt_tile);
    delete p;
    return cuda_fail(e, "vadb200_plan_create");
  }
  *out = p;
  return 0;
}

int vadb200_plan_destroy(vadb200_plan* p) {
  if (!p) return 0;
  cudaSetDevice(p->h->device);
  cudaFree(p->d_segs);
  cudaFree(p->d_counter);
  cudaFree(p->d_row_off);
  cudaFree(p->d_pcm_off);
  cudaFree(p->d_tiles);
  cudaFree(p->d_utt_tile);
  delete p;
  return 0;
}

int64_t vadb200_plan_total_rows(const vadb200_plan* p) { return p ? p->total_rows : -1; }
int64_t vadb200_plan_segment_frames(const vadb200_plan* p) { return p ? p->seg_frames : -1; }
int64_t vadb200_plan_segment_count(const vadb200_plan* p) { return p ? static_cast<int64_t>(p->segs.size()) : -1; }

int vadb200_set_plan_segment_frames(vadb200_handle* h, int frames) {
  if (!h || frames < 0 || frames > 2048 || (frames != 0 && (frames < 64 || frames % 32)))
    return fail(VADB200_E_INVALID, "segment length must be 0 (automatic) or a multiple of 32 in [64, 2048]");
  h->plan_seg_frames = frames;
  return 0;
}

int vadb200_plan_row_offsets(const vadb200_plan* p, int64_t* out) {
  if (!p || !out) return fail(VADB200_E_INVALID, "null argument");
  for (long long u = 0; u <= p->n_utt; ++u) out[u] = p->row_off[u];
  return 0;
}

static int check_pcm(const vadb200_plan* p, const void* pcm, int64_t pcm_len) {
  if (!p) return fail(VADB200_E_INVALID, "plan is null");
  if (p->total_rows > 0 && !pcm) return fail(VADB200_E_INVALID, "pcm is null");
  if (reinterpret_cast<uintptr_t>(pcm) & 15) return fail(VADB200_E_INVALID, "pcm must be 16-byte aligned");
  if (p->n_utt > 0 && pcm_len < p->offsets[p->n_utt - 1] + p->lengths[p->n_utt - 1])
    return fail(VADB200_E_INVALID, "pcm_len is smaller than the last utterance's end");
  return 0;
}

int vadb200_mfcc_packed(vadb200_plan* p, const int16_t* d_pcm, int64_t pcm_len, float* d_out, void* stream) {
  int rc = check_pcm(p, d_pcm, pcm_len);
  if (rc) return rc;
  if (p->mode == VADB200_MODE_VAD) return fail(VADB200_E_INVALID, "plan was created for MODE_VAD");
  if (p->total_rows > 0 && !d_out) return fail(VADB200_E_INVALID, "d_out is null");
  CU(cudaSetDevice(p->h->device));
  FusedParams fp = base_params(p);
  fp.pcm = d_pcm; fp.pcm_len = pcm_len; fp.rows = d_out;
  fp.seg_begin = 0; fp.seg_end = static_cast<int>(p->segs.size());
  return launch_fused(p, fp, fp.seg_end, static_cast<cudaStream_t>(stream));
}

int vadb200_vad_packed(vadb200_plan* p, const int16_t* d_pcm, int64_t pcm_len, uint8_t* d_labels, float* d_logits,
                       float* d_feats, int feat_mode, void* stream) {
  int rc = check_pcm(p, d_pcm, pcm_len);
  if (rc) return rc;
  if (p->mode != VADB200_MODE_VAD) return fail(VADB200_E_INVALID, "plan was not created for MODE_VAD");
  if (!p->h->have_ffn) return fail(VADB200_E_STATE, "FFN weights not set (vadb200_set_ffn_weights)");
  if (p->total_rows > 0 && !d_labels) return fail(VADB200_E_INVALID, "d_labels is null");
  if (feat_mode != VADB200_FEAT_ANALYSER && feat_mode != VADB200_FEAT_DATASET) return fail(VADB200_E_INVALID, "unknown feat_mode");
  CU(cudaSetDevice(p->h->device));
  FusedParams fp = base_params(p);
  fp.pcm = d_pcm; fp.pcm_len = pcm_len; fp.labels = d_labels; fp.logits = d_logits; fp.feats = d_feats;
  fp.feat_mode = feat_mode;
  fp.seg_begin = 0; fp.seg_end = static_cast<int>(p->segs.size());
  return launch_fused(p, fp, fp.seg_end, static_cast<cudaStream_t>(stream));
}

static int ensure_host_pipeline(vadb200_handle* h, long long stage_samples, long long rows, bool want_labels,
                                bool want_logits, long long row_floats) {
  if (!h->s_in) {
    CU(cudaStreamCreateWithFlags(&h->s_in, cudaStreamNonBlocking));
    CU(cudaStreamCreateWithFlags(&h->s_run, cudaStreamNonBlocking));
    CU(cudaStreamCreateWithFlags(&h->s_out, cudaStreamNonBlocking));
    for (int i = 0; i < kHostBufs; ++i) {
      CU(cudaEventCreateWithFlags(&h->ev_in[i], cudaEventDisableTiming));
      CU(cudaEventCreateWithFlags(&h->ev_done[i], cudaEventDisableTiming));
      CU(cudaEventCreateWithFlags(&h->ev_out[i], cudaEventDisableTiming));
    }
  }
  if (stage_samples > h->stage_cap) {
    for (int i = 0; i < kHostBufs; ++i) {
      cudaFree(h->d_stage[i]); h->d_stage[i] = nullptr;
      CU(cudaMalloc(&h->d_stage[i], stage_samples * sizeof(int16_t)));
    }
    h->stage_cap = stage_samples;
  }
  if (want_labels && rows > h->lab_cap) {
    for (int i = 0; i < kHostBufs; ++i) {
      cudaFree(h->d_lab[i]); h->d_lab[i] = nullptr;
      CU(cudaMalloc(&h->d_lab[i], rows));
    }
    h->lab_cap = rows;
  }
  if (want_logits && rows > h->lgt_cap) {
    for (int i = 0; i < kHostBufs; ++i) {
      cudaFree(h->d_lgt[i]); h->d_lgt[i] = nullptr;
      CU(cudaMalloc(&h->d_lgt[i], rows * 3 * sizeof(float)));
    }
    h->lgt_cap = rows;
  }
  if (row_floats > h->rows_cap) {
    for (int i = 0; i < kHostBufs; ++i) {
      cudaFree(h->d_rows[i]); h->d_rows[i] = nullptr;
      CU(cudaMalloc(&h->d_rows[i], row_floats * sizeof(float)));
    }
    h->rows_cap = row_floats;
  }
  return 0;
}

static int run_host_pipeline(vadb200_plan* p, const int16_t* h_pcm, int64_t pcm_len, uint8_t* h_labels, float* h_logits,
                             float* h_rows, int feat_mode) {
  vadb200_handle* h = p->h;
  if (p->total_rows == 0) return 0;
  if (p->n_utt > 0 && pcm_len < p->offsets[p->n_utt - 1] + p->lengths[p->n_utt - 1])
    return fail(VADB200_E_INVALID, "pcm_len is smaller than the last utterance's end");
  CU(cudaSetDevice(h->device));
  const long long width = p->mode == VADB200_MODE_VAD ? 0 : (p->mode == VADB200_MODE_MFCC ? kNCep : kNFeat);
  struct Chunk { long long u0, u1, s0, s1; };
  std::vector<Chunk> chunks;
  long long max_span = 0, max_rows = 0;
  for (long long u = 0; u < p->n_utt;) {
    Chunk c{u, u, p->offsets[u], 0};
    while (c.u1 < p->n_utt && (c.u1 == c.u0 || p->offsets[c.u1] + p->lengths[c.u1] - c.s0 <= h->host_chunk_samples)) ++c.u1;
    c.s1 = p->offsets[c.u1 - 1] + p->lengths[c.u1 - 1];
    max_span = std::max(max_span, c.s1 - c.s0);
    max_rows = std::max(max_rows, p->row_off[c.u1] - p->row_off[c.u0]);
    chunks.push_back(c);
    u = c.u1;
  }
  max_rows = std::max<long long>(max_rows, 1);
  int rc = ensure_host_pipeline(h, ((max_span + 7) & ~7ll) + 8, max_rows, h_labels != nullptr, h_logits != nullptr,
                                width * max_rows);
  if (rc) return rc;
  for (size_t i = 0; i < chunks.size(); ++i) {
    const Chunk& c = chunks[i];
    const int b = static_cast<int>(i % kHostBufs);
    const long long span = c.s1 - c.s0;
    const long long r0 = p->row_off[c.u0], nrows = p->row_off[c.u1] - r0;
    if (i >= kHostBufs) CU(cudaStreamWaitEvent(h->s_in, h->ev_done[b], 0));
    CU(cudaMemcpyAsync(h->d_stage[b], h_pcm + c.s0, span * sizeof(int16_t), cudaMemcpyHostToDevice, h->s_in));
    CU(cudaEventRecord(h->ev_in[b], h->s_in));
    CU(cudaStreamWaitEvent(h->s_run, h->ev_in[b], 0));
    if (i >= kHostBufs) CU(cudaStreamWaitEvent(h->s_run, h->ev_out[b], 0));
    FusedParams fp = base_params(p);
    fp.pcm = h->d_stage[b] - c.s0;
    fp.pcm_len = c.s1;
    fp.labels = h_labels ? h->d_lab[b] : nullptr;
    fp.logits = h_logits ? h->d_lgt[b] : nullptr;
    fp.rows = width ? h->d_rows[b] : nullptr;
    fp.row_base = r0;
    fp.feat_mode = feat_mode;
    fp.seg_begin = static_cast<int>(p->utt_seg[c.u0]);
    fp.seg_end = static_cast<int>(p->utt_seg[c.u1]);
    rc = launch_fused(p, fp, fp.seg_end - fp.seg_begin, h->s_run);
    if (rc) return rc;
    CU(cudaEventRecord(h->ev_done[b], h->s_run));
    CU(cudaStreamWaitEvent(h->s_out, h->ev_done[b], 0));
    if (nrows > 0) {
      if (h_labels) CU(cudaMemcpyAsync(h_labels + r0, h->d_lab[b], nrows, cudaMemcpyDeviceToHost, h->s_out));
      if (h_logits)
        CU(cudaMemcpyAsync(h_logits + r0 * 3, h->d_lgt[b], nrows * 3 * sizeof(float), cudaMemcpyDeviceToHost, h->s_out));
      if (width)
        CU(cudaMemcpyAsync(h_rows + r0 * width, h->d_rows[b], nrows * width * sizeof(float), cudaMemcpyDeviceToHost,
                           h->s_out));
    }
    CU(cudaEventRecord(h->ev_out[b], h->s_out));
  }
  CU(cudaStreamSynchronize(h->s_out));
  CU(cudaStreamSynchronize(h->s_run));
  return 0;
}

int vadb200_vad_host(vadb200_plan* p, const int16_t* h_pcm, int64_t pcm_len, uint8_t* h_labels, float* h_logits,
                     int feat_mode) {
  if (!p) return fail(VADB200_E_INVALID, "plan is null");
  if (p->mode != VADB200_MODE_VAD) return fail(VADB200_E_INVALID, "plan was not created for MODE_VAD");
  if (!p->h->have_ffn) return fail(VADB200_E_STATE, "FFN weights not set (vadb200_set_ffn_weights)");
  if (feat_mode != VADB200_FEAT_ANALYSER && feat_mode != VADB200_FEAT_DATASET) return fail(VADB200_E_INVALID, "unknown feat_mode");
  if (p->total_rows == 0) return 0;
  if (!h_pcm || !h_labels) return fail(VADB200_E_INVALID, "null argument");
  return run_host_pipeline(p, h_pcm, pcm_len, h_labels, h_logits, nullptr, feat_mode);
}

int vadb200_mfcc_host(vadb200_plan* p, const int16_t* h_pcm, int64_t pcm_len, float* h_out) {
  if (!p) return fail(VADB200_E_INVALID, "plan is null");
  if (p->mode == VADB200_MODE_VAD) return fail(VADB200_E_INVALID, "plan was created for MODE_VAD");
  if (p->total_rows == 0) return 0;
  if (!h_pcm || !h_out) return fail(VADB200_E_INVALID, "null argument");
  return run_host_pipeline(p, h_pcm, pcm_len, nullptr, nullptr, h_out, 0);
}

int vadb200_scale_rows(vadb200_handle* h, float* d_rows, int64_t n_rows, double* h_stats, void* stream) {
  if (!h || n_rows < 0) return fail(VADB200_E_INVALID, "bad argument");
  if (n_rows == 0) return 0;
  if (!d_rows) return fail(VADB200_E_INVALID, "d_rows is null");
  CU(cudaSetDevice(h->device));
  cudaStream_t st = static_cast<cudaStream_t>(stream);
  double* acc = nullptr;
  CU(cudaMallocAsync(&acc, 6 * sizeof(double), st));
  CU(cudaMemsetAsync(acc, 0, 6 * sizeof(double), st));
  const long long total = n_rows * kNFeat;
  const int grid = static_cast<int>(std::min<long long>((total + 255) / 256, 8ll * h->num_sms));
  for (int pass = 0; pass < 3; ++pass) {
    scale_rows_kernel<<<grid, 256, 0, st>>>(d_rows, n_rows, pass, acc);
    g_launches.fetch_add(1);
  }
  CU(cudaGetLastError());
  if (h_stats) {
    double raw[6];
    CU(cudaMemcpyAsync(raw, acc, sizeof(raw), cudaMemcpyDeviceToHost, st));
    CU(cudaStreamSynchronize(st));
    const double cnt = static_cast<double>(n_rows) * kNCep;
    for (int g = 0; g < 3; ++g) {
      h_stats[g] = raw[g] / cnt;
      h_stats[3 + g] = std::sqrt(raw[3 + g] / cnt);
    }
  }
  CU(cudaFreeAsync(acc, st));
  return 0;
}

int vadb200_ingest_pcm(vadb200_handle* h, const void* d_raw, int big_endian, const int64_t* d_src_start,
                       const int64_t* d_dst_start, const int64_t* d_len, int n_seg, int64_t max_len, int16_t* d_dst,
                       void* stream) {
  if (!h || n_seg < 0 || max_len < 0) return fail(VADB200_E_INVALID, "bad argument");
  if (n_seg == 0 || max_len == 0) return 0;
  if (!d_raw || !d_src_start || !d_dst_start || !d_len || !d_dst) return fail(VADB200_E_INVALID, "null argument");
  if (reinterpret_cast<uintptr_t>(d_raw) & 1) return fail(VADB200_E_INVALID, "raw sample stream must be 2-byte aligned");
  if (n_seg > 65535) return fail(VADB200_E_INVALID, "at most 65535 segments per call");
  CU(cudaSetDevice(h->device));
  const unsigned gx = static_cast<unsigned>(std::min<long long>((max_len + 255) / 256, 4ll * h->num_sms));
  static_assert(sizeof(long long) == sizeof(int64_t), "int64_t layout");
  ingest_kernel<<<dim3(gx, static_cast<unsigned>(n_seg)), 256, 0, static_cast<cudaStream_t>(stream)>>>(
      static_cast<const uint8_t*>(d_raw), big_endian, reinterpret_cast<const long long*>(d_src_start),
      reinterpret_cast<const long long*>(d_dst_start), reinterpret_cast<const long long*>(d_len), d_dst);
  g_launches.fetch_add(1);
  CU(cudaGetLastError());
  return 0;
}

static int frames_common(vadb200_handle* h, const float* d_frames, int64_t n, int frame_len, int what, float* d_out,
                         void* stream) {
  if (!h) return fail(VADB200_E_INVALID, "handle is null");
  if (n < 0 || frame_len < 1 || frame_len > kFftN) return fail(VADB200_E_INVALID, "need 1 <= frame_len <= 512, n >= 0");
  if (h->has_window && frame_len != kFrame) return fail(VADB200_E_INVALID, "a window needs frame_len == 400");
  if (n == 0) return 0;
  if (!d_frames || !d_out) return fail(VADB200_E_INVALID, "null argument");
  CU(cudaSetDevice(h->device));
  int rc = ensure_attrs(h);
  if (rc) return rc;
  cudaStream_t st = static_cast<cudaStream_t>(stream);
  rc = ensure_tables(h);
  if (rc) return rc;
  const unsigned grid = static_cast<unsigned>((n + kStepFrames - 1) / kStepFrames);
  const FrontEnd fe = frontend_on(h) ? frontend_of(h) : FrontEnd{nullptr, 0.0f};
  frames_kernel<<<grid, kThreads, kFramesSmemBytes, st>>>(d_frames, n, frame_len, what, d_out, h->d_tw, h->d_tw + 256, fe);
  g_launches.fetch_add(1);
  CU(cudaGetLastError());
  return 0;
}

int vadb200_spec_frames(vadb200_handle* h, const float* d_frames, int64_t n, int frame_len, float* d_spec, void* stream) {
  return frames_common(h, d_frames, n, frame_len, 0, d_spec, stream);
}
int vadb200_mfcc_frames(vadb200_handle* h, const float* d_frames, int64_t n, int frame_len, float* d_mfcc, void* stream) {
  return frames_common(h, d_frames, n, frame_len, 1, d_mfcc, stream);
}

int vadb200_mfcc_from_spec(vadb200_handle* h, const float* d_spec, int64_t n, float* d_mfcc, void* stream) {
  if (!h) return fail(VADB200_E_INVALID, "handle is null");
  if (n < 0) return fail(VADB200_E_INVALID, "n < 0");
  if (n == 0) return 0;
  if (!d_spec || !d_mfcc) return fail(VADB200_E_INVALID, "null argument");
  CU(cudaSetDevice(h->device));
  cudaStream_t st = static_cast<cudaStream_t>(stream);
  int rc = ensure_tables(h);
  if (rc) return rc;
  const unsigned grid = static_cast<unsigned>((n + kStepFrames - 1) / kStepFrames);
  spec_to_mfcc_kernel<<<grid, kThreads, 0, st>>>(d_spec, n, d_mfcc);
  g_launches.fetch_add(1);
  CU(cudaGetLastError());
  return 0;
}

int vadb200_vad_windows(vadb200_handle* h, const float* d_win, int64_t n, int feat_mode, uint8_t* d_labels,
                        float* d_logits, float* d_feats, void* stream) {
  if (!h) return fail(VADB200_E_INVALID, "handle is null");
  if (!h->have_ffn) return fail(VADB200_E_STATE, "FFN weights not set (vadb200_set_ffn_weights)");
  if (n < 0) return fail(VADB200_E_INVALID, "n < 0");
  if (n == 0) return 0;
  if (!d_win) return fail(VADB200_E_INVALID, "null argument");
  CU(cudaSetDevice(h->device));
  cudaStream_t st = static_cast<cudaStream_t>(stream);
  int rc = ensure_tables(h);
  if (rc) return rc;
  windows_kernel<<<static_cast<unsigned>((n + 127) / 128), 128, 0, st>>>(d_win, n, feat_mode, d_labels, d_logits, d_feats,
                                                                       h->par);
  g_launches.fetch_add(1);
  CU(cudaGetLastError());
  return 0;
}

int vadb200_ffn_predict(vadb200_handle* h, const float* d_x, int64_t n, uint8_t* d_labels, float* d_logits, void* stream) {
  if (!h) return fail(VADB200_E_INVALID, "handle is null");
  if (!h->have_ffn) return fail(VADB200_E_STATE, "FFN weights not set (vadb200_set_ffn_weights)");
  if (n < 0) return fail(VADB200_E_INVALID, "n < 0");
  if (n == 0) return 0;
  if (!d_x) return fail(VADB200_E_INVALID, "null argument");
  CU(cudaSetDevice(h->device));
  cudaStream_t st = static_cast<cudaStream_t>(stream);
  int rc = ensure_tables(h);
  if (rc) return rc;
  if (h->ffn_impl >= 2 && h->tc16_ok) {
    ffn_tc_rows_kernel<2><<<static_cast<unsigned>((n + 127) / 128), 128, kFfnTcSmemBytes, st>>>(
        d_x, n, h->d_tc16_blob, h->d_tc_blob, d_labels, d_logits, h->bias);
  } else if (h->ffn_impl >= 1) {
    ffn_tc_rows_kernel<1><<<static_cast<unsigned>((n + 127) / 128), 128, kFfnTcSmemBytes, st>>>(
        d_x, n, nullptr, h->d_tc_blob, d_labels, d_logits, h->bias);
  } else {
    ffn_rows_kernel<<<static_cast<unsigned>((n + 127) / 128), 128, 0, st>>>(d_x, n, d_labels, d_logits, h->par);
  }
  g_launches.fetch_add(1);
  CU(cudaGetLastError());
  return 0;
}

int vadb200_get_deltas(vadb200_handle* h, const float* d_a, const float* d_b, int64_t n, float* d_out, void* stream) {
  if (!h || n < 0) return fail(VADB200_E_INVALID, "bad argument");
  if (n == 0) return 0;
  if (!d_a || !d_b || !d_out) return fail(VADB200_E_INVALID, "null argument");
  CU(cudaSetDevice(h->device));
  elementwise_kernel<<<static_cast<unsigned>((n + 255) / 256), 256, 0, static_cast<cudaStream_t>(stream)>>>(0, d_a, d_b, n, 1, 0, d_out);
  g_launches.fetch_add(1);
  CU(cudaGetLastError());
  return 0;
}

int vadb200_lifter(vadb200_handle* h, const float* d_in, int64_t n_rows, int ncoef, int L, float* d_out, void* stream) {
  if (!h || n_rows < 0 || ncoef < 1) return fail(VADB200_E_INVALID, "bad argument");
  if (n_rows == 0) return 0;
  if (!d_in || !d_out) return fail(VADB200_E_INVALID, "null argument");
  CU(cudaSetDevice(h->device));
  const long long n = n_rows * ncoef;
  elementwise_kernel<<<static_cast<unsigned>((n + 255) / 256), 256, 0, static_cast<cudaStream_t>(stream)>>>(1, d_in, nullptr, n, ncoef, L, d_out);
  g_launches.fetch_add(1);
  CU(cudaGetLastError());
  return 0;
}

int vadb200_stream_bank_create(vadb200_handle* h, int n_streams, vadb200_bank** out) {
  if (!h || !out || n_streams < 1) return fail(VADB200_E_INVALID, "bad argument");
  *out = nullptr;
  CU(cudaSetDevice(h->device));
  vadb200_bank* b = new (std::nothrow) vadb200_bank();
  if (!b) return fail(VADB200_E_NOMEM, "host allocation failed");
  b->h = h; b->n = n_streams;
  cudaError_t e = cudaMalloc(&b->d_hist, static_cast<size_t>(n_streams) * 320 * sizeof(int16_t));
  if (e == cudaSuccess) e = cudaMalloc(&b->d_ring, static_cast<size_t>(n_streams) * 5 * kNCep * sizeof(float));
  if (e == cudaSuccess) e = cudaMalloc(&b->d_fed, static_cast<size_t>(n_streams) * sizeof(int));
  if (e == cudaSuccess) e = cudaMalloc(&b->d_prev, static_cast<size_t>(n_streams) * sizeof(int16_t));
  if (e != cudaSuccess) {
    cudaFree(b->d_hist); cudaFree(b->d_ring); cudaFree(b->d_fed); cudaFree(b->d_prev);
    delete b;
    return cuda_fail(e, "vadb200_stream_bank_create");
  }
  *out = b;
  int rc = vadb200_stream_bank_reset(b, nullptr);
  if (rc) return rc;
  CU(cudaDeviceSynchronize());
  return 0;
}

int vadb200_stream_bank_destroy(vadb200_bank* b) {
  if (!b) return 0;
  cudaSetDevice(b->h->device);
  cudaFree(b->d_hist); cudaFree(b->d_ring); cudaFree(b->d_fed); cudaFree(b->d_prev);
  delete b;
  return 0;
}

int vadb200_stream_bank_reset(vadb200_bank* b, void* stream) {
  if (!b) return fail(VADB200_E_INVALID, "bank is null");
  CU(cudaSetDevice(b->h->device));
  cudaStream_t st = static_cast<cudaStream_t>(stream);
  CU(cudaMemsetAsync(b->d_hist, 0, static_cast<size_t>(b->n) * 320 * sizeof(int16_t), st));
  CU(cudaMemsetAsync(b->d_ring, 0, static_cast<size_t>(b->n) * 5 * kNCep * sizeof(float), st));
  CU(cudaMemsetAsync(b->d_fed, 0, static_cast<size_t>(b->n) * sizeof(int), st));
  CU(cudaMemsetAsync(b->d_prev, 0, static_cast<size_t>(b->n) * sizeof(int16_t), st));
  return 0;
}

int vadb200_stream_feed(vadb200_bank* b, const int16_t* d_chunks, uint8_t* d_labels, float* d_logits, void* stream) {
  if (!b || !d_chunks || !d_labels) return fail(VADB200_E_INVALID, "null argument");
  vadb200_handle* h = b->h;
  if (!h->have_ffn) return fail(VADB200_E_STATE, "FFN weights not set (vadb200_set_ffn_weights)");
  if (reinterpret_cast<uintptr_t>(d_chunks) & 3) return fail(VADB200_E_INVALID, "chunks must be 4-byte aligned");
  CU(cudaSetDevice(h->device));
  int rc = ensure_attrs(h);
  if (rc) return rc;
  cudaStream_t st = static_cast<cudaStream_t>(stream);
  rc = ensure_tables(h);
  if (rc) return rc;
  BankParams bp;
  bp.n_streams = b->n; bp.hist = b->d_hist; bp.ring = b->d_ring; bp.fed = b->d_fed;
  bp.chunks = d_chunks; bp.labels = d_labels; bp.logits = d_logits;
  bp.tw1 = h->d_tw; bp.tw2 = h->d_tw + 256; bp.feat_mode = VADB200_FEAT_ANALYSER;
  bp.prev = b->d_prev;
  bp.fe = frontend_on(h) ? frontend_of(h) : FrontEnd{nullptr, 0.0f};
  stream_feed_kernel<<<(b->n + kStepFrames - 1) / kStepFrames, kThreads, kStreamSmemBytes, st>>>(bp, h->par);
  g_launches.fetch_add(1);
  CU(cudaGetLastError());
  return 0;
}

#if defined(VADB_DEBUG_HOOKS)
int vadb200_exp_fft(vadb200_plan* p, const int16_t* d_pcm, int64_t pcm_len, int minb, void* stream) {
  vadb200_handle* h = p->h;
  CU(cudaSetDevice(h->device));
  cudaStream_t st = static_cast<cudaStream_t>(stream);
  FusedParams fp = base_params(p);
  fp.pcm = d_pcm; fp.pcm_len = pcm_len; fp.seg_begin = 0; fp.seg_end = static_cast<int>(p->segs.size());
  fp.counter = p->d_counter + 2 * (p->launch_seq.fetch_add(1) % kPlanCounters);
  const int grid = std::min<int>(fp.seg_end, minb * h->num_sms);
#define VADB_EXP(M)                                                                                          \
  {                                                                                                          \
    CU(cudaFuncSetAttribute(exp_fft_kernel<M>, cudaFuncAttributeMaxDynamicSharedMemorySize, kExpSmemBytes)); \
    exp_fft_kernel<M><<<grid, kThreads, kExpSmemBytes, st>>>(fp, h->d_sink);                                 \
  }
  if (minb == 1) VADB_EXP(1) else if (minb == 2) VADB_EXP(2) else if (minb == 3) VADB_EXP(3) else VADB_EXP(4)
#undef VADB_EXP
  CU(cudaGetLastError());
  return 0;
}
#endif

int vadb200_trainer_create(vadb200_handle* h, int64_t max_batch, float lr, float rho, float eps, vadb200_trainer** out) {
  if (!h || !out || max_batch < 1) return fail(VADB200_E_INVALID, "bad argument");
  *out = nullptr;
  CU(cudaSetDevice(h->device));
  vadb200_trainer* t = new (std::nothrow) vadb200_trainer();
  if (!t) return fail(VADB200_E_NOMEM, "host allocation failed");
  t->h = h; t->max_batch = max_batch; t->lr = lr; t->rho = rho; t->eps = eps;
  const long long n_part = (max_batch + kTrainRows - 1) / kTrainRows;
  cudaError_t e = cudaMalloc(&t->d_state, 3 * kNParams * sizeof(float));
  if (e == cudaSuccess) e = cudaMemset(t->d_state, 0, 3 * kNParams * sizeof(float));
  if (e == cudaSuccess) e = cudaMalloc(&t->d_partial, n_part * (kNParams + 1) * sizeof(float));
  if (e == cudaSuccess) e = cudaMalloc(&t->d_loss, sizeof(float));
  if (e == cudaSuccess)
    e = cudaFuncSetAttribute(ffn_train_grad_kernel, cudaFuncAttributeMaxDynamicSharedMemorySize, kTrain2SmemBytes);
  if (e != cudaSuccess) {
    cudaFree(t->d_state); cudaFree(t->d_partial); cudaFree(t->d_loss);
    delete t;
    return cuda_fail(e, "vadb200_trainer_create");
  }
  if (h->have_ffn) {
    static_assert(sizeof(FfnParams) >= kNParams * sizeof(float), "FfnParams is the parameter vector");
    CU(cudaMemcpy(t->d_state, &h->par, kNParams * sizeof(float), cudaMemcpyHostToDevice));
  }
  *out = t;
  return 0;
}

int vadb200_trainer_destroy(vadb200_trainer* t) {
  if (!t) return 0;
  cudaSetDevice(t->h->device);
  cudaFree(t->d_state); cudaFree(t->d_partial); cudaFree(t->d_loss);
  delete t;
  return 0;
}

int vadb200_trainer_set_weights(vadb200_trainer* t, const float* W1, const float* b1, const float* W2, const float* b2,
                                const float* W3, const float* b3, const float* W4, const float* b4, int reset_optimizer) {
  if (!t || !W1 || !b1 || !W2 || !b2 || !W3 || !b3 || !W4 || !b4) return fail(VADB200_E_INVALID, "null argument");
  std::vector<float> v(kNParams);
  const float* src[8] = {W1, b1, W2, b2, W3, b3, W4, b4};
  const int off[9] = {kOffW1, kOffB1, kOffW2, kOffB2, kOffW3, kOffB3, kOffW4, kOffB4, kNParams};
  for (int i = 0; i < 8; ++i) std::memcpy(v.data() + off[i], src[i], (off[i + 1] - off[i]) * sizeof(float));
  CU(cudaSetDevice(t->h->device));
  CU(cudaDeviceSynchronize());
  CU(cudaMemcpy(t->d_state, v.data(), kNParams * sizeof(float), cudaMemcpyHostToDevice));
  if (reset_optimizer) CU(cudaMemset(t->d_state + kNParams, 0, 2 * kNParams * sizeof(float)));
  return 0;
}

int vadb200_trainer_get_weights(vadb200_trainer* t, float* W1, float* b1, float* W2, float* b2, float* W3, float* b3,
                                float* W4, float* b4) {
  if (!t || !W1 || !b1 || !W2 || !b2 || !W3 || !b3 || !W4 || !b4) return fail(VADB200_E_INVALID, "null argument");
  std::vector<float> v(kNParams);
  CU(cudaSetDevice(t->h->device));
  CU(cudaDeviceSynchronize());
  CU(cudaMemcpy(v.data(), t->d_state, kNParams * sizeof(float), cudaMemcpyDeviceToHost));
  float* dst[8] = {W1, b1, W2, b2, W3, b3, W4, b4};
  const int off[9] = {kOffW1, kOffB1, kOffW2, kOffB2, kOffW3, kOffB3, kOffW4, kOffB4, kNParams};
  for (int i = 0; i < 8; ++i) std::memcpy(dst[i], v.data() + off[i], (off[i + 1] - off[i]) * sizeof(float));
  return 0;
}

int vadb200_train_on_batch(vadb200_trainer* t, const float* d_x, const uint8_t* d_y, int64_t n, float* h_loss,
                           void* stream) {
  if (!t || n < 1 || !d_x || !d_y) return fail(VADB200_E_INVALID, "bad argument");
  if (n > t->max_batch) return fail(VADB200_E_INVALID, "batch larger than the trainer's max_batch");
  CU(cudaSetDevice(t->h->device));
  cudaStream_t st = static_cast<cudaStream_t>(stream);
  const int n_tiles = static_cast<int>((n + kTrainRows - 1) / kTrainRows);
  const int n_part = std::min(n_tiles, t->h->num_sms);
  ffn_train_grad_kernel<<<n_part, kTr2Threads, kTrain2SmemBytes, st>>>(t->d_state, d_x, d_y, n,
                                                                         1.0f / static_cast<float>(n), t->d_partial);
  ffn_train_update_kernel<<<(kNParams + 1 + 255) / 256, 256, 0, st>>>(t->d_state, t->d_state + kNParams,
                                                                       t->d_state + 2 * kNParams, t->d_partial, n_part,
                                                                       t->lr, t->rho, t->eps, t->d_loss);
  g_launches.fetch_add(2);
  CU(cudaGetLastError());
  ++t->steps;
  if (h_loss) {
    CU(cudaMemcpyAsync(h_loss, t->d_loss, sizeof(float), cudaMemcpyDeviceToHost, st));
    CU(cudaStreamSynchronize(st));
  }
  return 0;
}

int vadb200_synth_pcm(vadb200_handle* h, int16_t* d_out, int64_t n_utt, int64_t utt_samples, int64_t utt_stride,
                      uint32_t seed, int64_t first_utt, void* stream) {
  if (!h || !d_out || n_utt < 0 || utt_samples < 0 || utt_stride < utt_samples) return fail(VADB200_E_INVALID, "bad argument");
  if (n_utt == 0 || utt_samples == 0) return 0;
  CU(cudaSetDevice(h->device));
  const long long total = n_utt * utt_samples;
  const unsigned grid = static_cast<unsigned>(std::min<long long>((total + 255) / 256, 32ll * h->num_sms));
  synth_kernel<<<grid, 256, 0, static_cast<cudaStream_t>(stream)>>>(d_out, n_utt, utt_samples, utt_stride, seed, first_utt);
  g_launches.fetch_add(1);
  CU(cudaGetLastError());
  return 0;
}

int vadb200_fp32_peak(vadb200_handle* h, int variant, int iters, double* tflops_out) {
  if (!h || !tflops_out || iters < 1 || variant < 0 || variant > 6) return fail(VADB200_E_INVALID, "bad argument");
  CU(cudaSetDevice(h->device));
  int rc = ensure_tables(h);
  if (rc) return rc;
  cudaEvent_t e0, e1;
  CU(cudaEventCreate(&e0));
  CU(cudaEventCreate(&e1));
  const int grid = h->num_sms * 8;
  double best = 0.0;
  for (int rep = 0; rep < 5; ++rep) {
    CU(cudaEventRecord(e0, nullptr));
    if (variant == 0) fp32_peak_kernel<0><<<grid, 256>>>(h->d_sink, iters, 1.0000001f, 1e-9f);
    else if (variant == 1) fp32_peak_kernel<1><<<grid, 256>>>(h->d_sink, iters, 1.0000001f, 1e-9f);
    else if (variant == 2) fp32x2_peak_kernel<2><<<grid, 256>>>(h->d_sink, iters, 1.0000001f, 1e-9f);
    else if (variant == 3) fp32x2_peak_kernel<3><<<grid, 256>>>(h->d_sink, iters, 1.0000001f, 1e-9f);
    else if (variant == 4) fp32mix_peak_kernel<8><<<grid, 256>>>(h->d_sink, iters, 1.0000001f, 1e-9f);
    else if (variant == 5) fp32mix_peak_kernel<4><<<grid, 256>>>(h->d_sink, iters, 1.0000001f, 1e-9f);
    else fp32mix_peak_kernel<0><<<grid, 256>>>(h->d_sink, iters, 1.0000001f, 1e-9f);
    g_launches.fetch_add(1);
    CU(cudaEventRecord(e1, nullptr));
    CU(cudaEventSynchronize(e1));
    float ms = 0.f;
    CU(cudaEventElapsedTime(&ms, e0, e1));
    const double per_rep = variant <= 1 ? 2.0 * 16 : variant <= 3 ? 4.0 * 16
                         : variant == 4 ? 4.0 * 8 + 2.0 * 8 : variant == 5 ? 4.0 * 8 + 2.0 * 4 : 4.0 * 8;
    const double flops = per_rep * 8 * static_cast<double>(iters) * 256.0 * grid;
    if (rep > 0) best = std::max(best, flops / (ms * 1e-3) / 1e12);
  }
  cudaEventDestroy(e0);
  cudaEventDestroy(e1);
  *tflops_out = best;
  return 0;
}

namespace {
constexpr long long kWsAlign = 256;
long long ws_round(long long b) { return (b + kWsAlign - 1) / kWsAlign * kWsAlign; }
struct SpeechWs {
  long long counts, prefix, smoothed, total;
};
SpeechWs speech_ws(const vadb200_plan* p) {
  SpeechWs w;
  const long long nt = static_cast<long long>(p->tiles.size());
  w.counts = 0;
  w.prefix = ws_round(nt * static_cast<long long>(sizeof(int2)));
  w.smoothed = w.prefix + ws_round((nt + 1) * static_cast<long long>(sizeof(longlong2)));
  w.total = w.smoothed + ws_round(p->total_rows);
  return w;
}
bool misaligned(const void* ptr, uintptr_t a) { return (reinterpret_cast<uintptr_t>(ptr) & (a - 1)) != 0; }
}

int64_t vadb200_plan_max_speech_segments(const vadb200_plan* p) {
  if (!p || p->mode == VADB200_MODE_MFCC) return -1;
  return p->max_speech_segs;
}

int64_t vadb200_plan_speech_workspace_bytes(const vadb200_plan* p) {
  if (!p || p->mode == VADB200_MODE_MFCC) return -1;
  return speech_ws(p).total;
}

int vadb200_plan_speech_segments(vadb200_plan* p, const uint8_t* d_labels, int min_speech_rows, int min_silence_rows,
                                 int pad_rows, uint8_t* d_smoothed, int64_t* d_segments, int64_t* d_segment_offsets,
                                 int64_t* d_speech_offsets, void* d_workspace, int64_t workspace_bytes, void* stream) {
  if (!p) return fail(VADB200_E_INVALID, "plan is null");
  if (p->mode == VADB200_MODE_MFCC) return fail(VADB200_E_INVALID, "speech segments need a MODE_VAD or MODE_DATASET plan");
  for (int v : {min_speech_rows, min_silence_rows, pad_rows})
    if (v < 0 || v > kSpeechMaxParam) return fail(VADB200_E_INVALID, "row parameters must lie in [0, 1000]");
  const SpeechWs ws = speech_ws(p);
  if (!d_workspace || workspace_bytes < ws.total) return fail(VADB200_E_INVALID, "workspace is null or too small");
  if (misaligned(d_workspace, 16)) return fail(VADB200_E_INVALID, "workspace must be 16-byte aligned");
  if (!d_segment_offsets) return fail(VADB200_E_INVALID, "d_segment_offsets is null");
  if (p->total_rows > 0 && (!d_labels || !d_segments)) return fail(VADB200_E_INVALID, "d_labels / d_segments is null");
  if (misaligned(d_segments, 8) || misaligned(d_segment_offsets, 8) || misaligned(d_speech_offsets, 8))
    return fail(VADB200_E_INVALID, "segment and offset arrays must be 8-byte aligned");
  CU(cudaSetDevice(p->h->device));
  cudaStream_t st = static_cast<cudaStream_t>(stream);
  unsigned char* wsb = static_cast<unsigned char*>(d_workspace);
  int2* counts = reinterpret_cast<int2*>(wsb + ws.counts);
  longlong2* prefix = reinterpret_cast<longlong2*>(wsb + ws.prefix);
  uint8_t* sm = d_smoothed ? d_smoothed : wsb + ws.smoothed;
  const int n_tiles = static_cast<int>(p->tiles.size());
  const SmoothParams sp = smooth_params(min_speech_rows, min_silence_rows, pad_rows);
  if (n_tiles > 0) {
    speech_smooth_kernel<<<n_tiles, kSpeechThreads, smooth_smem_bytes(sp.H), st>>>(d_labels, p->d_tiles, p->d_row_off,
                                                                                 sp, sm, counts);
    g_launches.fetch_add(1);
  }
  speech_scan_kernel<<<1, kSpeechScanThreads, 0, st>>>(counts, n_tiles, prefix);
  g_launches.fetch_add(1);
  const long long utt_blocks = (p->n_utt + 1 + kSpeechThreads - 1) / kSpeechThreads;
  const unsigned grid = static_cast<unsigned>(std::max<long long>(n_tiles, utt_blocks));
  speech_segments_kernel<<<grid, kSpeechThreads, 0, st>>>(
      sm, p->d_tiles, p->d_row_off, prefix, n_tiles, p->d_utt_tile, p->n_utt, reinterpret_cast<long long*>(d_segments),
      reinterpret_cast<long long*>(d_segment_offsets), reinterpret_cast<long long*>(d_speech_offsets));
  g_launches.fetch_add(1);
  CU(cudaGetLastError());
  return 0;
}

int vadb200_plan_gather_speech(vadb200_plan* p, const int16_t* d_pcm, int64_t pcm_len, const int64_t* d_segments,
                               const int64_t* d_segment_offsets, const int64_t* d_speech_offsets, int16_t* d_out,
                               int64_t out_capacity, void* stream) {
  if (!p) return fail(VADB200_E_INVALID, "plan is null");
  if (p->mode == VADB200_MODE_MFCC) return fail(VADB200_E_INVALID, "speech segments need a MODE_VAD or MODE_DATASET plan");
  int rc = check_pcm(p, d_pcm, pcm_len);
  if (rc) return rc;
  if (out_capacity < 0) return fail(VADB200_E_INVALID, "out_capacity < 0");
  if (!d_segment_offsets || !d_speech_offsets) return fail(VADB200_E_INVALID, "offset arrays are null");
  if (p->total_rows > 0 && !d_segments) return fail(VADB200_E_INVALID, "d_segments is null");
  if (out_capacity > 0 && !d_out) return fail(VADB200_E_INVALID, "d_out is null");
  if (misaligned(d_out, 16)) return fail(VADB200_E_INVALID, "d_out must be 16-byte aligned");
  if (misaligned(d_segments, 8) || misaligned(d_segment_offsets, 8) || misaligned(d_speech_offsets, 8))
    return fail(VADB200_E_INVALID, "segment and offset arrays must be 8-byte aligned");
  if (p->total_rows == 0 || out_capacity == 0) return 0;
  CU(cudaSetDevice(p->h->device));
  const long long max_hops = p->total_rows;
  const unsigned grid = static_cast<unsigned>(std::max<long long>(1, std::min<long long>(8ll * p->h->num_sms, max_hops)));
  speech_gather_kernel<<<grid, kSpeechThreads, 0, static_cast<cudaStream_t>(stream)>>>(
      d_pcm, p->d_pcm_off, p->n_utt, reinterpret_cast<const long long*>(d_segments),
      reinterpret_cast<const long long*>(d_segment_offsets), reinterpret_cast<const long long*>(d_speech_offsets), d_out,
      out_capacity);
  g_launches.fetch_add(1);
  CU(cudaGetLastError());
  return 0;
}

}
```

### vad_b200/runtime.py

```python
import ctypes as C

import numpy as np
import torch

from . import _lib
from ._lib import check

MODE_MFCC, MODE_DATASET, MODE_VAD = 0, 1, 2
FEAT_ANALYSER, FEAT_DATASET = 0, 1
FFN_KEYS = ("W1", "b1", "W2", "b2", "W3", "b3", "W4", "b4")
FFN_SHAPES = {"W1": (39, 64), "b1": (64,), "W2": (64, 32), "b2": (32,), "W3": (32, 16), "b3": (16,),
              "W4": (16, 3), "b4": (3,)}


def _ptr(t):
    return C.c_void_p(t.data_ptr()) if t is not None else C.c_void_p(0)


def _stream(device):
    return C.c_void_p(torch.cuda.current_stream(device).cuda_stream)


def frames_for_length(n_samples):
    return int(_lib.load().vadb200_frames_for_length(int(n_samples)))


def outputs_for_length(n_samples):
    return int(_lib.load().vadb200_outputs_for_length(int(n_samples)))


def glorot_ffn(seed=0):
    rng = np.random.default_rng(seed)
    w = {}
    dims = (39, 64, 32, 16, 3)
    for i in range(4):
        lim = np.sqrt(6.0 / (dims[i] + dims[i + 1]))
        w["W%d" % (i + 1)] = rng.uniform(-lim, lim, size=(dims[i], dims[i + 1])).astype(np.float32)
        w["b%d" % (i + 1)] = np.zeros(dims[i + 1], dtype=np.float32)
    return w


def load_ffn_npz(path):
    z = np.load(path)
    return {k: np.asarray(z[k], dtype=np.float32) for k in FFN_KEYS}


class Handle(object):

    def __init__(self, device=None, ffn_weights=None):
        self.lib = _lib.load()
        if not torch.cuda.is_available():
            raise RuntimeError("vad_b200 needs a CUDA device (sm_100a); there is no CPU fallback")
        self.device = torch.device("cuda", torch.cuda.current_device() if device is None else int(
            device.index if isinstance(device, torch.device) else device))
        torch.cuda.init()
        with torch.cuda.device(self.device):
            torch.zeros(1, device=self.device)
        self._h = C.c_void_p()
        cfg = _lib.Config()
        self.lib.vadb200_default_config(C.byref(cfg))
        check(self.lib.vadb200_create(C.byref(cfg), self.device.index, C.byref(self._h)))
        self.has_ffn = False
        if ffn_weights is not None:
            self.set_ffn_weights(ffn_weights)

    def close(self):
        if getattr(self, "_h", None) is not None and self._h:
            self.lib.vadb200_destroy(self._h)
            self._h = C.c_void_p()

    def __del__(self):
        try:
            self.close()
        except Exception:
            pass

    @property
    def stream(self):
        return _stream(self.device)

    def filterbank(self):
        out = np.empty((26, 256), dtype=np.float64)
        check(self.lib.vadb200_get_filterbank(self._h, out.ctypes.data_as(C.c_void_p)))
        return out

    def set_ffn_weights(self, w):
        arrs = []
        for k in FFN_KEYS:
            a = np.ascontiguousarray(np.asarray(w[k], dtype=np.float32))
            if a.shape != FFN_SHAPES[k]:
                raise ValueError("FFN weight %s must have shape %r, got %r" % (k, FFN_SHAPES[k], a.shape))
            arrs.append(a)
        check(self.lib.vadb200_set_ffn_weights(self._h, *[a.ctypes.data_as(C.c_void_p) for a in arrs]))
        self.has_ffn = True

    def set_ffn_impl(self, impl):
        impl = {"fp32": 0, "tc": 1, "tc16": 2}.get(impl, impl)
        check(self.lib.vadb200_set_ffn_impl(self._h, int(impl)))

    @property
    def ffn_impl(self):
        return int(self.lib.vadb200_get_ffn_impl(self._h))

    def set_frontend(self, preemph=0.0, window=None):
        if isinstance(window, str):
            if window != "hamming":
                raise ValueError("window must be an array of 400 weights, 'hamming' or None")
            window = np.hamming(400)
        win = None
        if window is not None:
            win = np.ascontiguousarray(np.asarray(window, dtype=np.float32))
            if win.shape != (400,):
                raise ValueError("window must have 400 weights, got shape %r" % (win.shape,))
        check(self.lib.vadb200_set_frontend(self._h, float(preemph),
                                            win.ctypes.data_as(C.c_void_p) if win is not None else C.c_void_p(0)))

    def frontend(self):
        a = C.c_float()
        has = C.c_int()
        win = np.empty(400, dtype=np.float32)
        check(self.lib.vadb200_get_frontend(self._h, C.byref(a), win.ctypes.data_as(C.c_void_p), C.byref(has)))
        return float(a.value), (win if has.value else None)

    def set_decision_threshold(self, p=None):
        check(self.lib.vadb200_set_decision_threshold(self._h, 0.0 if p is None else float(p)))

    def decision_threshold(self):
        v = float(self.lib.vadb200_get_decision_threshold(self._h))
        return v if v > 0.0 else None

    def _frames_tensor(self, frames):
        t = torch.as_tensor(np.asarray(frames, dtype=np.float32) if not torch.is_tensor(frames) else frames)
        t = t.to(device=self.device, dtype=torch.float32)
        if t.dim() == 1:
            t = t[None]
        return t.contiguous()

    def spec_frames(self, frames):
        t = self._frames_tensor(frames)
        out = torch.empty((t.shape[0], 256), dtype=torch.float32, device=self.device)
        check(self.lib.vadb200_spec_frames(self._h, _ptr(t), t.shape[0], t.shape[1], _ptr(out), self.stream))
        return out

    def mfcc_frames(self, frames):
        t = self._frames_tensor(frames)
        out = torch.empty((t.shape[0], 13), dtype=torch.float32, device=self.device)
        check(self.lib.vadb200_mfcc_frames(self._h, _ptr(t), t.shape[0], t.shape[1], _ptr(out), self.stream))
        return out

    def mfcc_from_spec(self, spec):
        t = self._frames_tensor(spec)
        if t.shape[1] != 256:
            raise ValueError("spectrum must have fft_n/2 = 256 bins")
        out = torch.empty((t.shape[0], 13), dtype=torch.float32, device=self.device)
        check(self.lib.vadb200_mfcc_from_spec(self._h, _ptr(t), t.shape[0], _ptr(out), self.stream))
        return out

    def vad_windows(self, windows, feat_mode=FEAT_ANALYSER, want_feats=False):
        t = torch.as_tensor(windows).to(device=self.device, dtype=torch.float32).contiguous().reshape(-1, 5, 13)
        n = t.shape[0]
        labels = torch.empty((n,), dtype=torch.uint8, device=self.device)
        logits = torch.empty((n, 3), dtype=torch.float32, device=self.device)
        feats = torch.empty((n, 39), dtype=torch.float32, device=self.device) if want_feats else None
        check(self.lib.vadb200_vad_windows(self._h, _ptr(t), n, feat_mode, _ptr(labels), _ptr(logits), _ptr(feats),
                                           self.stream))
        return labels, logits, feats

    def ffn_predict(self, x):
        t = torch.as_tensor(x).to(device=self.device, dtype=torch.float32).contiguous().reshape(-1, 39)
        n = t.shape[0]
        labels = torch.empty((n,), dtype=torch.uint8, device=self.device)
        logits = torch.empty((n, 3), dtype=torch.float32, device=self.device)
        check(self.lib.vadb200_ffn_predict(self._h, _ptr(t), n, _ptr(labels), _ptr(logits), self.stream))
        return labels, logits

    def synth_pcm(self, n_utt, utt_samples, seed=1234, first_utt=0, utt_stride=None, out=None):
        utt_stride = utt_samples if utt_stride is None else utt_stride
        if out is None:
            out = torch.zeros((n_utt * utt_stride + 8,), dtype=torch.int16, device=self.device)
        check(self.lib.vadb200_synth_pcm(self._h, _ptr(out), n_utt, utt_samples, utt_stride, seed & 0xFFFFFFFF,
                                         first_utt, self.stream))
        return out

    def fp32_peak(self, variant=0, iters=4096):
        v = C.c_double()
        check(self.lib.vadb200_fp32_peak(self._h, variant, iters, C.byref(v)))
        return v.value

    def set_host_chunk_samples(self, samples):
        check(self.lib.vadb200_set_host_chunk_samples(self._h, int(samples)))

    def set_plan_segment_frames(self, frames):
        check(self.lib.vadb200_set_plan_segment_frames(self._h, int(frames)))

    def scale_rows(self, rows, want_stats=True):
        if not (torch.is_tensor(rows) and rows.is_cuda and rows.dtype == torch.float32 and rows.is_contiguous()
                and rows.dim() == 2 and rows.shape[1] == 39):
            raise TypeError("rows must be a contiguous [n, 39] float32 CUDA tensor")
        stats = np.zeros(6, dtype=np.float64) if want_stats else None
        check(self.lib.vadb200_scale_rows(self._h, _ptr(rows), rows.shape[0],
                                          stats.ctypes.data_as(C.c_void_p) if want_stats else C.c_void_p(0),
                                          self.stream))
        return stats

    def ingest_pcm(self, raw, src_start, dst_start, lengths, out, big_endian=False):
        src = torch.as_tensor(np.asarray(src_start, dtype=np.int64)).to(self.device)
        dst = torch.as_tensor(np.asarray(dst_start, dtype=np.int64)).to(self.device)
        ln_host = np.asarray(lengths, dtype=np.int64)
        ln = torch.as_tensor(ln_host).to(self.device)
        if ln_host.size == 0:
            return out
        check(self.lib.vadb200_ingest_pcm(self._h, _ptr(raw), 1 if big_endian else 0, _ptr(src), _ptr(dst), _ptr(ln),
                                          int(ln_host.size), int(ln_host.max()), _ptr(out), self.stream))
        return out


class Plan(object):

    def __init__(self, handle, offsets, lengths, mode):
        self.handle = handle
        self.lib = handle.lib
        self.mode = mode
        self.offsets = np.ascontiguousarray(offsets, dtype=np.int64)
        self.lengths = np.ascontiguousarray(lengths, dtype=np.int64)
        if self.offsets.shape != self.lengths.shape or self.offsets.ndim != 1:
            raise ValueError("offsets and lengths must be 1-D arrays of equal length")
        self.n_utt = int(self.offsets.shape[0])
        self._p = C.c_void_p()
        check(self.lib.vadb200_plan_create(handle._h, self.offsets.ctypes.data_as(C.c_void_p),
                                           self.lengths.ctypes.data_as(C.c_void_p), self.n_utt, mode,
                                           C.byref(self._p)))
        self.total_rows = int(self.lib.vadb200_plan_total_rows(self._p))
        self.segment_frames = int(self.lib.vadb200_plan_segment_frames(self._p))
        self.segment_count = int(self.lib.vadb200_plan_segment_count(self._p))
        self.row_offsets = np.empty(self.n_utt + 1, dtype=np.int64)
        check(self.lib.vadb200_plan_row_offsets(self._p, self.row_offsets.ctypes.data_as(C.c_void_p)))

    def close(self):
        if getattr(self, "_p", None) is not None and self._p:
            self.lib.vadb200_plan_destroy(self._p)
            self._p = C.c_void_p()

    def __del__(self):
        try:
            self.close()
        except Exception:
            pass

    def _check_pcm(self, pcm):
        if not (torch.is_tensor(pcm) and pcm.dtype == torch.int16 and pcm.is_contiguous() and pcm.dim() == 1):
            raise TypeError("pcm must be a contiguous 1-D torch.int16 tensor")

    def mfcc(self, pcm, out=None):
        self._check_pcm(pcm)
        width = 13 if self.mode == MODE_MFCC else 39
        if out is None:
            out = torch.empty((self.total_rows, width), dtype=torch.float32, device=pcm.device)
        check(self.lib.vadb200_mfcc_packed(self._p, _ptr(pcm), pcm.numel(), _ptr(out), self.handle.stream))
        return out

    def vad(self, pcm, labels=None, want_logits=False, want_feats=False, feat_mode=FEAT_ANALYSER, logits=None):
        self._check_pcm(pcm)
        dev = pcm.device
        if labels is None:
            labels = torch.empty((self.total_rows,), dtype=torch.uint8, device=dev)
        if logits is None and want_logits:
            logits = torch.empty((self.total_rows, 3), dtype=torch.float32, device=dev)
        feats = torch.empty((self.total_rows, 39), dtype=torch.float32, device=dev) if want_feats else None
        check(self.lib.vadb200_vad_packed(self._p, _ptr(pcm), pcm.numel(), _ptr(labels), _ptr(logits), _ptr(feats),
                                          feat_mode, self.handle.stream))
        return labels, logits, feats

    def mfcc_host(self, pcm_host, out_host=None):
        if not (torch.is_tensor(pcm_host) and pcm_host.dtype == torch.int16 and not pcm_host.is_cuda):
            raise TypeError("pcm_host must be a CPU torch.int16 tensor")
        width = 13 if self.mode == MODE_MFCC else 39
        if out_host is None:
            out_host = torch.empty((self.total_rows, width), dtype=torch.float32).pin_memory()
        check(self.lib.vadb200_mfcc_host(self._p, _ptr(pcm_host), pcm_host.numel(), _ptr(out_host)))
        return out_host

    def vad_host(self, pcm_host, labels_host=None, logits_host=None, feat_mode=FEAT_ANALYSER):
        if not (torch.is_tensor(pcm_host) and pcm_host.dtype == torch.int16 and not pcm_host.is_cuda):
            raise TypeError("pcm_host must be a CPU torch.int16 tensor")
        if labels_host is None:
            labels_host = torch.empty((self.total_rows,), dtype=torch.uint8).pin_memory()
        check(self.lib.vadb200_vad_host(self._p, _ptr(pcm_host), pcm_host.numel(), _ptr(labels_host),
                                        _ptr(logits_host), feat_mode))
        return labels_host, logits_host


    def speech_segments(self, labels, min_speech_ms=0, min_silence_ms=0, pad_ms=0, want_smoothed=False):
        if not (torch.is_tensor(labels) and labels.is_cuda and labels.dtype == torch.uint8 and labels.is_contiguous()
                and labels.dim() == 1 and labels.numel() == self.total_rows):
            raise TypeError("labels must be a contiguous uint8 CUDA tensor of the plan's %d rows" % self.total_rows)
        rows = [speech_ms_to_rows(v) for v in (min_speech_ms, min_silence_ms, pad_ms)]
        dev = labels.device
        ws_bytes = int(self.lib.vadb200_plan_speech_workspace_bytes(self._p))
        if ws_bytes < 0:
            raise ValueError("speech segments need a MODE_VAD or MODE_DATASET plan")
        ws = getattr(self, "_speech_ws", None)
        if ws is None or ws.numel() < ws_bytes or ws.device != dev:
            ws = self._speech_ws = torch.empty((max(ws_bytes, 16),), dtype=torch.uint8, device=dev)
        max_segs = int(self.lib.vadb200_plan_max_speech_segments(self._p))
        segs = torch.empty((max(max_segs, 1), 2), dtype=torch.int64, device=dev)
        offs = torch.empty((2, self.n_utt + 1), dtype=torch.int64, device=dev)
        smoothed = torch.empty((self.total_rows,), dtype=torch.uint8, device=dev) if want_smoothed else None
        check(self.lib.vadb200_plan_speech_segments(self._p, _ptr(labels), rows[0], rows[1], rows[2], _ptr(smoothed),
                                                    _ptr(segs), _ptr(offs[0]), _ptr(offs[1]), _ptr(ws), ws_bytes,
                                                    self.handle.stream))
        offs_h = offs.cpu().numpy()
        return segs[:int(offs_h[0, -1])], offs_h[0].copy(), offs_h[1].copy(), smoothed

    def gather_speech(self, pcm, segments, segment_offsets, speech_offsets, out=None):
        self._check_pcm(pcm)
        dev = pcm.device
        so = torch.as_tensor(np.asarray(segment_offsets, dtype=np.int64)).to(dev)
        sp_h = np.asarray(speech_offsets, dtype=np.int64)
        sp = torch.as_tensor(sp_h).to(dev)
        if so.numel() != self.n_utt + 1 or sp.numel() != self.n_utt + 1:
            raise ValueError("offsets must have n_utt + 1 entries")
        segs = segments if segments.numel() else torch.zeros((1, 2), dtype=torch.int64, device=dev)
        total = int(sp_h[-1])
        if out is None:
            out = torch.empty((total,), dtype=torch.int16, device=dev)
        check(self.lib.vadb200_plan_gather_speech(self._p, _ptr(pcm), pcm.numel(), _ptr(segs.contiguous()), _ptr(so),
                                                  _ptr(sp), _ptr(out), out.numel(), self.handle.stream))
        return out


def speech_ms_to_rows(ms):
    ms = float(ms)
    if not ms >= 0.0:
        raise ValueError("durations must be >= 0 ms")
    rows = int(np.ceil(ms / 10.0))
    if rows > 1000:
        raise ValueError("durations must be at most 10000 ms (1000 rows)")
    return rows


class StreamBankHandle(object):
    def __init__(self, handle, n_streams):
        self.handle = handle
        self.lib = handle.lib
        self.n = int(n_streams)
        self._b = C.c_void_p()
        check(self.lib.vadb200_stream_bank_create(handle._h, self.n, C.byref(self._b)))

    def close(self):
        if getattr(self, "_b", None) is not None and self._b:
            self.lib.vadb200_stream_bank_destroy(self._b)
            self._b = C.c_void_p()

    def __del__(self):
        try:
            self.close()
        except Exception:
            pass

    def reset(self):
        check(self.lib.vadb200_stream_bank_reset(self._b, self.handle.stream))

    def feed_ptr(self, chunks_ptr, labels_ptr, logits_ptr=0, stream=None):
        check(self.lib.vadb200_stream_feed(self._b, C.c_void_p(chunks_ptr), C.c_void_p(labels_ptr),
                                           C.c_void_p(logits_ptr), stream if stream is not None else self.handle.stream))


_default = {}


def default_handle(device=None):
    idx = torch.cuda.current_device() if device is None else int(device)
    if idx not in _default:
        _default[idx] = Handle(idx)
    return _default[idx]


def _handle_get_deltas(self, a, b):
    ta = torch.as_tensor(np.asarray(a, dtype=np.float32) if not torch.is_tensor(a) else a).to(
        device=self.device, dtype=torch.float32).contiguous()
    tb = torch.as_tensor(np.asarray(b, dtype=np.float32) if not torch.is_tensor(b) else b).to(
        device=self.device, dtype=torch.float32).contiguous()
    if ta.shape != tb.shape:
        raise ValueError("operands must have equal shapes")
    out = torch.empty_like(ta)
    check(self.lib.vadb200_get_deltas(self._h, _ptr(ta), _ptr(tb), ta.numel(), _ptr(out), self.stream))
    return out


def _handle_lifter(self, cepstra, L=22):
    t = torch.as_tensor(np.asarray(cepstra, dtype=np.float32) if not torch.is_tensor(cepstra) else cepstra).to(
        device=self.device, dtype=torch.float32).contiguous()
    ncoef = int(t.shape[0]) if t.dim() == 1 else int(t.shape[-1])
    out = torch.empty_like(t)
    check(self.lib.vadb200_lifter(self._h, _ptr(t), t.numel() // max(ncoef, 1), ncoef, int(L), _ptr(out), self.stream))
    return out


Handle.get_deltas = _handle_get_deltas
Handle.lifter = _handle_lifter
```

Baseline: 20.22 million.

## Pack multiple utterance pieces into shared work units with prefetched unit tables

Replaces per-segment work items with work units that pack up to 16 utterance pieces side by side in one frame-slot range. This cuts the partially filled steps and per-segment scheduling overhead on short utterances. The next unit is claimed and its first load issued during the last step of the current unit, which overlaps the unit transition. The cost is per-piece lookup logic in the output paths, gap slots between pieces, and more shared memory for double-buffered piece tables.

```diff
diff --git a/include/vadb200.h b/include/vadb200.h
--- a/include/vadb200.h
+++ b/include/vadb200.h
@@ -72,6 +72,8 @@
 int vadb200_plan_row_offsets(const vadb200_plan* p, int64_t* h_out );
 int64_t vadb200_plan_segment_frames(const vadb200_plan* p);
 int64_t vadb200_plan_segment_count(const vadb200_plan* p);
+int64_t vadb200_plan_unit_count(const vadb200_plan* p);
+int64_t vadb200_plan_frame_slots(const vadb200_plan* p);
 int vadb200_set_plan_segment_frames(vadb200_handle* h, int frames);
 
 int vadb200_mfcc_packed(vadb200_plan* p, const int16_t* d_pcm, int64_t pcm_len, float* d_out,
diff --git a/vad_b200/_lib.py b/vad_b200/_lib.py
--- a/vad_b200/_lib.py
+++ b/vad_b200/_lib.py
@@ -42,6 +42,8 @@
     "vadb200_plan_row_offsets": (C.c_int, [_P, _P]),
     "vadb200_plan_segment_frames": (_I64, [_P]),
     "vadb200_plan_segment_count": (_I64, [_P]),
+    "vadb200_plan_unit_count": (_I64, [_P]),
+    "vadb200_plan_frame_slots": (_I64, [_P]),
     "vadb200_set_plan_segment_frames": (C.c_int, [_P, C.c_int]),
     "vadb200_mfcc_host": (C.c_int, [_P, _P, _I64, _P]),
     "vadb200_plan_max_speech_segments": (_I64, [_P]),
diff --git a/vad_b200/csrc/vad_kernels.cuh b/vad_b200/csrc/vad_kernels.cuh
--- a/vad_b200/csrc/vad_kernels.cuh
+++ b/vad_b200/csrc/vad_kernels.cuh
@@ -4,6 +4,7 @@
 
 #include "vad_core.cuh"
 #include "ffn_tc.cuh"
+#include "vad_pack.h"
 
 namespace vadb {
 
@@ -27,19 +28,16 @@
 constexpr int kOffTw2 = kOffTw1 + 256 * 8;
 constexpr int kOffBar = kOffTw2 + 128 * 8;
 constexpr int kOffSeg = kOffBar + 48;
-constexpr int kFusedSmemBytes = kOffSeg + 16;
+constexpr int kOffPcs = kOffSeg + 16;
+constexpr int kPcTableBytes = kUnitPieces * (4 + 8 + 8);
+constexpr int kFusedSmemBytes = kOffPcs + 2 * kPcTableBytes;
 constexpr int kBlockStepsTc = 4;
 static_assert(kTcBlobBytes <= kWarps * 2 * kExchFrame * 8 + kP2Bytes, "weight blob must fit exch + P");
 static_assert(kBlockSteps * kStepFrames * kNFeat * 4 + 16 <= kWarps * 2 * kExchFrame * 8 + kP2Bytes,
               "dataset-row staging tile must fit exch + P");
 static_assert(2 * (kFusedSmemBytes + 1024) <= 233472, "two CTAs per SM");
 
-struct Segment {
-  long long pcm_start;
-  long long out_start;
-  int n_frames;
-  int cont;
-};
+static_assert(kPackHop == kHop && kPackFrame == kFrame, "vad_pack.h frame geometry");
 
 struct FrontEnd {
   const cf2* win;
@@ -55,8 +53,9 @@
 struct FusedParams {
   const int16_t* pcm;
   long long pcm_len;
-  const Segment* segs;
-  int seg_begin, seg_end;
+  const Piece* pieces;
+  const int* unit_piece;
+  int unit_begin, unit_end;
   int* counter;
   const cf2* tw1;
   const cf2* tw2;
@@ -245,6 +244,12 @@
 constexpr int kStageOffFe = 8;
 static_assert(kStageSamples + kStageOffFe <= kStagePad, "front-end stage offset must fit the PCM buffer");
 
+__device__ __forceinline__ int piece_of_slot(const int* s_pc, int np, int c) {
+  int j = 0;
+  while (j + 1 < np && (s_pc[j + 1] & 0xffff) <= c) ++j;
+  return j;
+}
+
 template <int MODE, int TC, bool FE>
 __device__ __forceinline__ void fused_body(const FusedParams& p, const typename FfnArgOf<MODE, TC>::type& ffn,
                                            const FrontEnd& fe, const int tid) {
@@ -287,44 +292,79 @@
   }
 
   unsigned gstep = 0;
-  Segment seg{};
+  unsigned gunit = 0;
+  auto pc_rng = [&](unsigned tb) { return reinterpret_cast<int*>(smem + kOffPcs + tb * kPcTableBytes); };
+  auto pc_out = [&](unsigned tb) {
+    return reinterpret_cast<long long*>(smem + kOffPcs + tb * kPcTableBytes + kUnitPieces * 4);
+  };
+  auto pc_pcm = [&](unsigned tb) {
+    return reinterpret_cast<long long*>(smem + kOffPcs + tb * kPcTableBytes + kUnitPieces * 12);
+  };
   const P2Store p2store(s_P, col_of_halfwarp(warp, h), t);
   __syncthreads();
   warp_arrive(&s_bar[4], lane);
 
 
-  auto issue_load = [&](int step, int buf) {
-    const long long start = seg.pcm_start + static_cast<long long>(step) * (kStepFrames * kHop);
-    const long long avail = p.pcm_len - start;
-    const int nsmp = avail >= kStageSamples ? kStageSamples : (avail > 0 ? static_cast<int>(avail) : 0);
-    const int bulk = (nsmp * 2) & ~15;
-    int16_t* dst = s_pcm + buf * kStagePad + kStageOff;
-    if (tid == 0) {
-      mbar_arrive_expect_tx(&s_bar[buf], static_cast<uint32_t>(bulk));
-      if (bulk) bulk_g2s(dst, p.pcm + start, static_cast<uint32_t>(bulk), &s_bar[buf]);
-    }
-    const int tail0 = bulk >> 1;
-    if (tid < nsmp - tail0) dst[tail0 + tid] = p.pcm[start + tail0 + tid];
-    if (FE && tid == 31) dst[-1] = (step > 0 || seg.cont) ? p.pcm[start - 1] : int16_t(0);
+  auto issue_pieces = [&](bool mine, int first, int end, long long pcm_start, bool cont, int step, int buf) {
+    const int s0 = step * kStepFrames;
+    const int a = max(first, s0), b = min(end, s0 + kStepFrames);
+    const bool act = mine && a < b;
+    const uint32_t bytes = act ? static_cast<uint32_t>(((b - a - 1) * kHop + kFrame) * 2) : 0u;
+    const uint32_t total = __reduce_add_sync(0xffffffffu, bytes);
+    if (lane == 0) mbar_arrive_expect_tx(&s_bar[buf], total);
+    __syncwarp();
+    if (act) {
+      int16_t* dst = s_pcm + buf * kStagePad + kStageOff + (a - s0) * kHop;
+      const long long src = pcm_start + static_cast<long long>(a - first) * kHop;
+      bulk_g2s(dst, p.pcm + src, bytes, &s_bar[buf]);
+      if (FE) dst[-1] = (a > first || cont) ? p.pcm[src - 1] : int16_t(0);
+    }
   };
+  auto issue_load = [&](const int* s_pc, const long long* s_pcm, int np, int step, int buf) {
+    const bool mine = lane < np;
+    const int r = mine ? s_pc[lane] : 0;
+    const long long pc = mine ? s_pcm[lane] : 0;
+    issue_pieces(mine, r & 0xffff, r >> 16, pc & ~1ll, (pc & 1) != 0, step, buf);
+  };
+  auto take_unit = [&](int claimed, unsigned tb, int buf) {
+    const int ui = p.unit_begin + __shfl_sync(0xffffffffu, claimed, 0);
+    int np = 0;
+    Piece q{};
+    if (ui < p.unit_end) {
+      const int pc0 = p.unit_piece[ui];
+      np = p.unit_piece[ui + 1] - pc0;
+      if (lane < np) {
+        q = p.pieces[pc0 + lane];
+        pc_rng(tb)[lane] = q.slot | ((q.slot + q.n_frames) << 16);
+        pc_out(tb)[lane] = q.out_start - p.row_base;
+        pc_pcm(tb)[lane] = q.pcm_start | q.cont;
+      }
+      issue_pieces(lane < np, q.slot, q.slot + q.n_frames, q.pcm_start, q.cont != 0, 0, buf);
+    }
+    if (lane == 0) {
+      s_seg[0] = ui;
+      s_seg[1] = np;
+    }
+  };
+  if (warp == 0) take_unit(lane == 0 ? atomicAdd(p.counter, 1) : 0, 0, 0);
 
   for (;;) {
     __syncthreads();
-    if (tid == 0) *s_seg = p.seg_begin + atomicAdd(p.counter, 1);
-    __syncthreads();
-    const int si = *s_seg;
-    if (si >= p.seg_end) break;
-    seg = p.segs[si];
-    const int n = seg.n_frames;
+    const int ui = s_seg[0], np = s_seg[1];
+    if (ui >= p.unit_end) break;
+    const unsigned tb = gunit++ & 1;
+    const int* s_pc = pc_rng(tb);
+    const long long* s_pc_out = pc_out(tb);
+    const long long* s_pc_pcm = pc_pcm(tb);
+    const int n = s_pc[np - 1] >> 16;
     const int nsteps = (n + kStepFrames - 1) / kStepFrames;
     int out_done = (MODE == 0) ? 0 : 2;
     bool dct_pending = false;
-    if (nsteps > 0 && warp == 0) issue_load(0, gstep & 1);
-    __syncthreads();
 
     for (int s = 0; s < nsteps; ++s, ++gstep) {
       const int buf = gstep & 1;
-      if (s + 1 < nsteps && warp == 0) issue_load(s + 1, buf ^ 1);
+      const bool last = s + 1 == nsteps;
+      if (warp == 0 && !last) issue_load(s_pc, s_pc_pcm, np, s + 1, buf ^ 1);
       mbar_wait(&s_bar[buf], (gstep >> 1) & 1);
 
       const uint32_t par = gstep & 1;
@@ -359,6 +399,8 @@
         mbar_wait(&s_bar[4], par);
       }
       warp_arrive(&s_bar[5], lane);
+      int claimed = 0;
+      if (last && tid == 0) claimed = atomicAdd(p.counter, 1);
 
       if (dct_pending) dct_step(s - 1);
       mbar_wait(&s_bar[5], par);
@@ -366,6 +408,7 @@
       if (!(VADB_DBG(p) & 2))
         mel2_run_dispatch<kP2Pitch, 32>(warp, s_P + 2 * lane, s_logE + (s & 1) * kLogEFloats + lane);
       warp_arrive(&s_bar[4], lane);
+      if (last && warp == 0) take_unit(claimed, tb ^ 1u, buf ^ 1);
       const int computed = min((s + 1) * kStepFrames, n);
       const bool block_now = (((s + 1) % kBlk) == 0 || s == nsteps - 1) && !(VADB_DBG(p) & 8);
       const bool tc_now = TC && block_now && (computed - 2 - out_done) > 0;
@@ -385,22 +428,26 @@
       if (block_now) {
         __syncthreads();
         if (MODE == 0) {
-          float* dst = p.rows + (seg.out_start - p.row_base + out_done) * kNCep;
-          const int first = out_done;
-          flush_flat(dst, (computed - out_done) * kNCep, tid, [&](int j, float (&v)[4], int cnt) {
-            int fr = j / kNCep, cf = j - fr * kNCep;
-#pragma unroll
-            for (int i = 0; i < 4; ++i) {
-              if (i < cnt) v[i] = s_ring[ring_idx(cf, (first + fr) % kRing, kRing)];
-              if (++cf == kNCep) { cf = 0; ++fr; }
-            }
-          });
+          for (int j = piece_of_slot(s_pc, np, out_done); j < np && (s_pc[j] & 0xffff) < computed; ++j) {
+            const int first = max(out_done, s_pc[j] & 0xffff), last = min(computed, s_pc[j] >> 16);
+            if (first >= last) continue;
+            float* dst = p.rows + (s_pc_out[j] + (first - (s_pc[j] & 0xffff))) * kNCep;
+            flush_flat(dst, (last - first) * kNCep, tid, [&](int jj, float (&v)[4], int cnt) {
+              int fr = jj / kNCep, cf = jj - fr * kNCep;
+#pragma unroll
+              for (int i = 0; i < 4; ++i) {
+                if (i < cnt) v[i] = s_ring[ring_idx(cf, (first + fr) % kRing, kRing)];
+                if (++cf == kNCep) { cf = 0; ++fr; }
+              }
+            });
+          }
           out_done = computed;
         } else if (MODE == 1) {
           const int n_valid = computed - 2 - out_done;
           if (n_valid > 0) {
-            float* dst = p.rows + (seg.out_start - p.row_base + (out_done - 2)) * kNFeat;
-            float* stage = reinterpret_cast<float*>(smem + kOffExch) + ((reinterpret_cast<uintptr_t>(dst) & 15u) >> 2);
+            const int j0 = piece_of_slot(s_pc, np, out_done);
+            float* dst0 = p.rows + (s_pc_out[j0] + (out_done - 2 - (s_pc[j0] & 0xffff))) * kNFeat;
+            float* stage = reinterpret_cast<float*>(smem + kOffExch) + ((reinterpret_cast<uintptr_t>(dst0) & 15u) >> 2);
             if (tid < n_valid) {
               float xa[24], xb[24];
               window_features_pairs<0, 4, kRing, 24>(s_ring, out_done + tid, 1, xa);
@@ -415,22 +462,31 @@
               }
             }
             __syncthreads();
-            flush_flat(dst, n_valid * kNFeat, tid, [&](int j, float (&v)[4], int cnt) {
-              if (cnt == 4) {
-                const float4 q = *reinterpret_cast<const float4*>(stage + j);
-                v[0] = q.x; v[1] = q.y; v[2] = q.z; v[3] = q.w;
-              } else {
-#pragma unroll
-                for (int i = 0; i < 4; ++i)
-                  if (i < cnt) v[i] = stage[j + i];
-              }
-            });
+            for (int j = j0; j < np && (s_pc[j] & 0xffff) + 2 < computed - 2; ++j) {
+              const int st = s_pc[j] & 0xffff;
+              const int first = max(out_done, st + 2), last = min(computed - 2, (s_pc[j] >> 16) - 2);
+              if (first >= last) continue;
+              float* dst = p.rows + (s_pc_out[j] + (first - 2 - st)) * kNFeat;
+              const float* src = stage + (first - out_done) * kNFeat;
+              const bool vec = ((reinterpret_cast<uintptr_t>(dst) ^ reinterpret_cast<uintptr_t>(src)) & 15u) == 0;
+              flush_flat(dst, (last - first) * kNFeat, tid, [&](int jj, float (&v)[4], int cnt) {
+                if (cnt == 4 && vec) {
+                  const float4 q = *reinterpret_cast<const float4*>(src + jj);
+                  v[0] = q.x; v[1] = q.y; v[2] = q.z; v[3] = q.w;
+                } else {
+#pragma unroll
+                  for (int i = 0; i < 4; ++i)
+                    if (i < cnt) v[i] = src[jj + i];
+                }
+              });
+            }
             __syncthreads();
           }
           out_done = max(out_done, computed - 2);
         } else if (!TC) {
           const int c = out_done + tid;
-          if (c <= computed - 3) {
+          const int j = piece_of_slot(s_pc, np, c), st = s_pc[j] & 0xffff;
+          if (c <= computed - 3 && c >= st + 2 && c + 3 <= (s_pc[j] >> 16)) {
             float r[5][kNCep];
 #pragma unroll
             for (int d = 0; d < 5; ++d) {
@@ -439,7 +495,7 @@
               for (int k = 0; k < kNCep; ++k) r[d][k] = s_ring[ring_idx(k, col, kRing)];
             }
             if constexpr (MODE == 2 && TC == 0)
-              classify_row(ffn, r, p.feat_mode, p.labels, p.logits, p.feats, seg.out_start - p.row_base + (c - 2),
+              classify_row(ffn, r, p.feat_mode, p.labels, p.logits, p.feats, s_pc_out[j] + (c - 2 - st),
                            FE ? ffn.thresh : 0.0f);
           }
           out_done = max(out_done, computed - 2);
@@ -454,8 +510,10 @@
               if (p.dbg_ts && blockIdx.x == 0 && tid == 0 && dbg_n < 64) ts = p.dbg_ts + 16 * dbg_n;
 #endif
               if (ts) ts[0] = clock64();
-              const bool valid = fr < n_valid;
-              const int c = out_done + (valid ? fr : 0);
+              const int c = out_done + (fr < n_valid ? fr : 0);
+              const int j = piece_of_slot(s_pc, np, c), st = s_pc[j] & 0xffff;
+              const bool valid = fr < n_valid && c >= st + 2 && c + 3 <= (s_pc[j] >> 16);
+              const long long row = s_pc_out[j] + (c - 2 - st);
               const uint32_t tl = tm_base + (static_cast<uint32_t>(32 * (warp & 3)) << 16);
               float xl[24], logit[kNCls];
               bool ok_half = true;
@@ -471,7 +529,6 @@
               if constexpr (TC == 2) tc16_store_a1_half(tl, hidx, xl);
               else tc_store_a1_half(tl, hidx, xl);
               if (p.feats && valid) {
-                const long long row = seg.out_start - p.row_base + (c - 2);
                 const int k0 = hidx ? 8 : 0, nk = hidx ? 5 : 8;
 #pragma unroll
                 for (int k = 0; k < 8; ++k)
@@ -494,7 +551,6 @@
                   logit[0] = logit[1] = logit[2] = NAN;
                   lab = 0;
                 }
-                const long long row = seg.out_start - p.row_base + (c - 2);
                 p.labels[row] = lab;
                 if (p.logits) {
                   p.logits[row * 3 + 0] = logit[0];
@@ -642,7 +698,7 @@
   }
   unsigned gstep = 0;
   float acc = 0.0f;
-  Segment seg;
+  Piece seg;
   auto issue_load = [&](int step, int buf) {
     const long long start = seg.pcm_start + static_cast<long long>(step) * (kStepFrames * kHop);
     const long long avail = p.pcm_len - start;
@@ -655,12 +711,13 @@
   };
   for (;;) {
     __syncthreads();
-    if (tid == 0) *s_seg = p.seg_begin + atomicAdd(p.counter, 1);
+    if (tid == 0) *s_seg = p.unit_begin + atomicAdd(p.counter, 1);
     __syncthreads();
     const int si = *s_seg;
-    if (si >= p.seg_end) break;
-    seg = p.segs[si];
-    const int nsteps = (seg.n_frames + kStepFrames - 1) / kStepFrames;
+    if (si >= p.unit_end) break;
+    seg = p.pieces[p.unit_piece[si]];
+    const Piece last = p.pieces[p.unit_piece[si + 1] - 1];
+    const int nsteps = (last.slot + last.n_frames + kStepFrames - 1) / kStepFrames;
     issue_load(0, gstep & 1);
     __syncthreads();
     for (int s = 0; s < nsteps; ++s, ++gstep) {
diff --git a/vad_b200/csrc/vad_pack.h b/vad_b200/csrc/vad_pack.h
--- /dev/null
+++ b/vad_b200/csrc/vad_pack.h
@@ -0,0 +1,78 @@
+#pragma once
+
+#include <algorithm>
+#include <vector>
+
+namespace vadb {
+
+constexpr int kUnitPieces = 16;
+constexpr int kPackGap = 2;
+constexpr int kPackHop = 160;
+constexpr int kPackFrame = 400;
+
+struct Piece {
+  long long pcm_start;
+  long long out_start;
+  int slot;
+  int n_frames;
+  int cont;
+  int pad;
+};
+
+struct PackLayout {
+  std::vector<Piece> pieces;
+  std::vector<int> unit_piece;
+};
+
+inline void pack_units(const long long* offs, const long long* row_off, long long n_utt, int halo,
+                       long long unit_slots, PackLayout& L) {
+  L.pieces.clear();
+  L.unit_piece.assign(1, 0);
+  long long used = 0;
+  int npc = 0;
+  auto close_unit = [&] {
+    if (npc) L.unit_piece.push_back(static_cast<int>(L.pieces.size()));
+    used = 0;
+    npc = 0;
+  };
+  for (long long u = 0; u < n_utt; ++u) {
+    const long long r = row_off[u + 1] - row_off[u];
+    for (long long o = 0; o < r;) {
+      const long long first = npc ? used + kPackGap : 0;
+      const long long room = unit_slots - first, need = r - o + halo;
+      if (npc && (npc == kUnitPieces || room < halo + 1 || (need > room && need <= unit_slots))) {
+        close_unit();
+        continue;
+      }
+      const long long take = std::min(need, room);
+      Piece q;
+      q.pcm_start = offs[u] + kPackHop * o;
+      q.out_start = row_off[u] + o;
+      q.slot = static_cast<int>(first);
+      q.n_frames = static_cast<int>(take);
+      q.cont = o > 0 ? 1 : 0;
+      q.pad = 0;
+      L.pieces.push_back(q);
+      ++npc;
+      used = first + take;
+      o += take - halo;
+    }
+  }
+  close_unit();
+}
+
+inline long long unit_pcm_begin(const PackLayout& L, long long u) {
+  const Piece& q = L.pieces[L.unit_piece[u]];
+  return q.pcm_start - (q.cont ? 8 : 0);
+}
+inline long long unit_pcm_end(const PackLayout& L, long long u) {
+  const Piece& q = L.pieces[L.unit_piece[u + 1] - 1];
+  return q.pcm_start + static_cast<long long>(q.n_frames - 1) * kPackHop + kPackFrame;
+}
+inline long long unit_row_begin(const PackLayout& L, long long u) { return L.pieces[L.unit_piece[u]].out_start; }
+inline long long unit_row_end(const PackLayout& L, long long u, int halo) {
+  const Piece& q = L.pieces[L.unit_piece[u + 1] - 1];
+  return q.out_start + q.n_frames - halo;
+}
+
+}
diff --git a/vad_b200/csrc/vadb200.cu b/vad_b200/csrc/vadb200.cu
--- a/vad_b200/csrc/vadb200.cu
+++ b/vad_b200/csrc/vadb200.cu
@@ -87,9 +87,10 @@
   vadb200_handle* h = nullptr;
   int mode = 0;
   long long n_utt = 0;
-  std::vector<long long> offsets, lengths, row_off, utt_seg;
-  std::vector<Segment> segs;
-  Segment* d_segs = nullptr;
+  std::vector<long long> offsets, lengths, row_off;
+  PackLayout pack;
+  Piece* d_pieces = nullptr;
+  int* d_unit_piece = nullptr;
   int* d_counter = nullptr;
   std::atomic<unsigned> launch_seq{0};
   long long total_rows = 0;
@@ -157,9 +158,9 @@
 bool frontend_on(const vadb200_handle* h) { return h->preemph != 0.0f || h->has_window; }
 FrontEnd frontend_of(const vadb200_handle* h) { return FrontEnd{h->d_win, h->preemph}; }
 
-int launch_fused(vadb200_plan* p, FusedParams fp, int n_segs, cudaStream_t st) {
+int launch_fused(vadb200_plan* p, FusedParams fp, int n_units, cudaStream_t st) {
   vadb200_handle* h = p->h;
-  if (n_segs <= 0) return 0;
+  if (n_units <= 0) return 0;
   int rc = ensure_attrs(h);
   if (rc) return rc;
   rc = ensure_tables(h);
@@ -171,7 +172,7 @@
 #else
   const int per_sm = 2;
 #endif
-  const int grid = std::min(n_segs, per_sm * h->num_sms);
+  const int grid = std::min(n_units, per_sm * h->num_sms);
   const bool fe = frontend_on(h) || (p->mode == VADB200_MODE_VAD && h->par.thresh > 0.0f);
   const FrontEnd fea = frontend_of(h);
   if (fe) {
@@ -212,10 +213,13 @@
   return 0;
 }
 
+int plan_units(const vadb200_plan* p) { return static_cast<int>(p->pack.unit_piece.size()) - 1; }
+
 FusedParams base_params(vadb200_plan* p) {
   FusedParams fp;
   std::memset(&fp, 0, sizeof(fp));
-  fp.segs = p->d_segs;
+  fp.pieces = p->d_pieces;
+  fp.unit_piece = p->d_unit_piece;
   fp.counter = p->d_counter;
   fp.tw1 = p->h->d_tw;
   fp.tw2 = p->h->d_tw + 256;
@@ -438,7 +442,6 @@
   p->offsets.assign(offs, offs + n_utt);
   p->lengths.assign(lens, lens + n_utt);
   p->row_off.resize(n_utt + 1);
-  p->utt_seg.resize(n_utt + 1);
   long long rows = 0, prev_end = 0;
   for (long long u = 0; u < n_utt; ++u) {
     if (offs[u] < 0 || (offs[u] & 7) || lens[u] < 0 || offs[u] < prev_end) {
@@ -455,34 +458,26 @@
   long long seg_frames = h->plan_seg_frames;
   if (seg_frames <= 0) {
     const long long want = rows / (16ll * 2 * h->num_sms) + halo;
-    seg_frames = want <= 64 ? 64 : std::min<long long>(2048, ((want + 127) / 128) * 128);
+    seg_frames = want <= 64 ? 64 : std::min<long long>(4096, ((want + 127) / 128) * 128);
   }
   p->seg_frames = seg_frames;
-  const long long seg_rows = seg_frames - halo;
-  for (long long u = 0; u < n_utt; ++u) {
-    p->utt_seg[u] = static_cast<long long>(p->segs.size());
-    const long long r = p->row_off[u + 1] - p->row_off[u];
-    for (long long o = 0; o < r; o += seg_rows) {
-      Segment s;
-      s.pcm_start = offs[u] + kHop * o;
-      s.out_start = p->row_off[u] + o;
-      s.n_frames = static_cast<int>(std::min(seg_rows, r - o) + halo);
-      s.cont = o > 0 ? 1 : 0;
-      p->segs.push_back(s);
-    }
-  }
-  p->utt_seg[n_utt] = static_cast<long long>(p->segs.size());
-  if (p->segs.size() > 0x7fffffffull) {
+  pack_units(p->offsets.data(), p->row_off.data(), n_utt, halo, seg_frames, p->pack);
+  const size_t n_pieces = p->pack.pieces.size();
+  if (p->pack.unit_piece.size() > 0x7fffffffull) {
     delete p;
-    return fail(VADB200_E_INVALID, "too many segments");
+    return fail(VADB200_E_INVALID, "too many work units");
   }
   cudaError_t e = cudaSetDevice(h->device);
   if (e == cudaSuccess) e = cudaMalloc(&p->d_counter, 2 * kPlanCounters * sizeof(int));
   if (e == cudaSuccess) e = cudaMemset(p->d_counter, 0, 2 * kPlanCounters * sizeof(int));
-  if (e == cudaSuccess && !p->segs.empty()) {
-    e = cudaMalloc(&p->d_segs, p->segs.size() * sizeof(Segment));
+  if (e == cudaSuccess && n_pieces > 0) {
+    e = cudaMalloc(&p->d_pieces, n_pieces * sizeof(Piece));
     if (e == cudaSuccess)
-      e = cudaMemcpy(p->d_segs, p->segs.data(), p->segs.size() * sizeof(Segment), cudaMemcpyHostToDevice);
+      e = cudaMemcpy(p->d_pieces, p->pack.pieces.data(), n_pieces * sizeof(Piece), cudaMemcpyHostToDevice);
+    const size_t nu = p->pack.unit_piece.size();
+    if (e == cudaSuccess) e = cudaMalloc(&p->d_unit_piece, nu * sizeof(int));
+    if (e == cudaSuccess)
+      e = cudaMemcpy(p->d_unit_piece, p->pack.unit_piece.data(), nu * sizeof(int), cudaMemcpyHostToDevice);
   }
   if (mode != VADB200_MODE_MFCC) {
     p->utt_tile.resize(n_utt + 1);
@@ -513,7 +508,7 @@
     }
   }
   if (e != cudaSuccess) {
-    cudaFree(p->d_counter); cudaFree(p->d_segs);
+    cudaFree(p->d_counter); cudaFree(p->d_pieces); cudaFree(p->d_unit_piece);
     cudaFree(p->d_row_off); cudaFree(p->d_pcm_off); cudaFree(p->d_tiles); cudaFree(p->d_utt_tile);
     delete p;
     return cuda_fail(e, "vadb200_plan_create");
@@ -525,7 +520,8 @@
 int vadb200_plan_destroy(vadb200_plan* p) {
   if (!p) return 0;
   cudaSetDevice(p->h->device);
-  cudaFree(p->d_segs);
+  cudaFree(p->d_pieces);
+  cudaFree(p->d_unit_piece);
   cudaFree(p->d_counter);
   cudaFree(p->d_row_off);
   cudaFree(p->d_pcm_off);
@@ -537,11 +533,21 @@
 
 int64_t vadb200_plan_total_rows(const vadb200_plan* p) { return p ? p->total_rows : -1; }
 int64_t vadb200_plan_segment_frames(const vadb200_plan* p) { return p ? p->seg_frames : -1; }
-int64_t vadb200_plan_segment_count(const vadb200_plan* p) { return p ? static_cast<int64_t>(p->segs.size()) : -1; }
+int64_t vadb200_plan_segment_count(const vadb200_plan* p) { return p ? static_cast<int64_t>(p->pack.pieces.size()) : -1; }
+int64_t vadb200_plan_unit_count(const vadb200_plan* p) { return p ? plan_units(p) : -1; }
+int64_t vadb200_plan_frame_slots(const vadb200_plan* p) {
+  if (!p) return -1;
+  long long slots = 0;
+  for (int u = 0; u < plan_units(p); ++u) {
+    const Piece& q = p->pack.pieces[p->pack.unit_piece[u + 1] - 1];
+    slots += (q.slot + q.n_frames + 31) / 32 * 32;
+  }
+  return slots;
+}
 
 int vadb200_set_plan_segment_frames(vadb200_handle* h, int frames) {
-  if (!h || frames < 0 || frames > 2048 || (frames != 0 && (frames < 64 || frames % 32)))
-    return fail(VADB200_E_INVALID, "segment length must be 0 (automatic) or a multiple of 32 in [64, 2048]");
+  if (!h || frames < 0 || frames > 4096 || (frames != 0 && (frames < 64 || frames % 32)))
+    return fail(VADB200_E_INVALID, "segment length must be 0 (automatic) or a multiple of 32 in [64, 4096]");
   h->plan_seg_frames = frames;
   return 0;
 }
@@ -569,8 +575,8 @@
   CU(cudaSetDevice(p->h->device));
   FusedParams fp = base_params(p);
   fp.pcm = d_pcm; fp.pcm_len = pcm_len; fp.rows = d_out;
-  fp.seg_begin = 0; fp.seg_end = static_cast<int>(p->segs.size());
-  return launch_fused(p, fp, fp.seg_end, static_cast<cudaStream_t>(stream));
+  fp.unit_begin = 0; fp.unit_end = plan_units(p);
+  return launch_fused(p, fp, fp.unit_end, static_cast<cudaStream_t>(stream));
 }
 
 int vadb200_vad_packed(vadb200_plan* p, const int16_t* d_pcm, int64_t pcm_len, uint8_t* d_labels, float* d_logits,
@@ -585,8 +591,8 @@
   FusedParams fp = base_params(p);
   fp.pcm = d_pcm; fp.pcm_len = pcm_len; fp.labels = d_labels; fp.logits = d_logits; fp.feats = d_feats;
   fp.feat_mode = feat_mode;
-  fp.seg_begin = 0; fp.seg_end = static_cast<int>(p->segs.size());
-  return launch_fused(p, fp, fp.seg_end, static_cast<cudaStream_t>(stream));
+  fp.unit_begin = 0; fp.unit_end = plan_units(p);
+  return launch_fused(p, fp, fp.unit_end, static_cast<cudaStream_t>(stream));
 }
 
 static int ensure_host_pipeline(vadb200_handle* h, long long stage_samples, long long rows, bool want_labels,
@@ -640,15 +646,18 @@
     return fail(VADB200_E_INVALID, "pcm_len is smaller than the last utterance's end");
   CU(cudaSetDevice(h->device));
   const long long width = p->mode == VADB200_MODE_VAD ? 0 : (p->mode == VADB200_MODE_MFCC ? kNCep : kNFeat);
-  struct Chunk { long long u0, u1, s0, s1; };
+  struct Chunk { long long u0, u1, s0, s1, r0, r1; };
   std::vector<Chunk> chunks;
   long long max_span = 0, max_rows = 0;
-  for (long long u = 0; u < p->n_utt;) {
-    Chunk c{u, u, p->offsets[u], 0};
-    while (c.u1 < p->n_utt && (c.u1 == c.u0 || p->offsets[c.u1] + p->lengths[c.u1] - c.s0 <= h->host_chunk_samples)) ++c.u1;
-    c.s1 = p->offsets[c.u1 - 1] + p->lengths[c.u1 - 1];
+  const int halo = p->mode == VADB200_MODE_MFCC ? 0 : 4;
+  const long long n_units = plan_units(p);
+  for (long long u = 0; u < n_units;) {
+    Chunk c{u, u, unit_pcm_begin(p->pack, u), 0, unit_row_begin(p->pack, u), 0};
+    while (c.u1 < n_units && (c.u1 == c.u0 || unit_pcm_end(p->pack, c.u1) - c.s0 <= h->host_chunk_samples)) ++c.u1;
+    c.s1 = unit_pcm_end(p->pack, c.u1 - 1);
+    c.r1 = unit_row_end(p->pack, c.u1 - 1, halo);
     max_span = std::max(max_span, c.s1 - c.s0);
-    max_rows = std::max(max_rows, p->row_off[c.u1] - p->row_off[c.u0]);
+    max_rows = std::max(max_rows, c.r1 - c.r0);
     chunks.push_back(c);
     u = c.u1;
   }
@@ -660,7 +669,7 @@
     const Chunk& c = chunks[i];
     const int b = static_cast<int>(i % kHostBufs);
     const long long span = c.s1 - c.s0;
-    const long long r0 = p->row_off[c.u0], nrows = p->row_off[c.u1] - r0;
+    const long long r0 = c.r0, nrows = c.r1 - c.r0;
     if (i >= kHostBufs) CU(cudaStreamWaitEvent(h->s_in, h->ev_done[b], 0));
     CU(cudaMemcpyAsync(h->d_stage[b], h_pcm + c.s0, span * sizeof(int16_t), cudaMemcpyHostToDevice, h->s_in));
     CU(cudaEventRecord(h->ev_in[b], h->s_in));
@@ -674,9 +683,9 @@
     fp.rows = width ? h->d_rows[b] : nullptr;
     fp.row_base = r0;
     fp.feat_mode = feat_mode;
-    fp.seg_begin = static_cast<int>(p->utt_seg[c.u0]);
-    fp.seg_end = static_cast<int>(p->utt_seg[c.u1]);
-    rc = launch_fused(p, fp, fp.seg_end - fp.seg_begin, h->s_run);
+    fp.unit_begin = static_cast<int>(c.u0);
+    fp.unit_end = static_cast<int>(c.u1);
+    rc = launch_fused(p, fp, fp.unit_end - fp.unit_begin, h->s_run);
     if (rc) return rc;
     CU(cudaEventRecord(h->ev_done[b], h->s_run));
     CU(cudaStreamWaitEvent(h->s_out, h->ev_done[b], 0));
@@ -943,9 +952,9 @@
   CU(cudaSetDevice(h->device));
   cudaStream_t st = static_cast<cudaStream_t>(stream);
   FusedParams fp = base_params(p);
-  fp.pcm = d_pcm; fp.pcm_len = pcm_len; fp.seg_begin = 0; fp.seg_end = static_cast<int>(p->segs.size());
+  fp.pcm = d_pcm; fp.pcm_len = pcm_len; fp.unit_begin = 0; fp.unit_end = plan_units(p);
   fp.counter = p->d_counter + 2 * (p->launch_seq.fetch_add(1) % kPlanCounters);
-  const int grid = std::min<int>(fp.seg_end, minb * h->num_sms);
+  const int grid = std::min<int>(fp.unit_end, minb * h->num_sms);
 #define VADB_EXP(M)                                                                                          \
   {                                                                                                          \
     CU(cudaFuncSetAttribute(exp_fft_kernel<M>, cudaFuncAttributeMaxDynamicSharedMemorySize, kExpSmemBytes)); \
diff --git a/vad_b200/runtime.py b/vad_b200/runtime.py
--- a/vad_b200/runtime.py
+++ b/vad_b200/runtime.py
@@ -233,6 +233,8 @@
         self.total_rows = int(self.lib.vadb200_plan_total_rows(self._p))
         self.segment_frames = int(self.lib.vadb200_plan_segment_frames(self._p))
         self.segment_count = int(self.lib.vadb200_plan_segment_count(self._p))
+        self.unit_count = int(self.lib.vadb200_plan_unit_count(self._p))
+        self.frame_slots = int(self.lib.vadb200_plan_frame_slots(self._p))
         self.row_offsets = np.empty(self.n_utt + 1, dtype=np.int64)
         check(self.lib.vadb200_plan_row_offsets(self._p, self.row_offsets.ctypes.data_as(C.c_void_p)))
 
```

Result: slower. 19.23 million (median of 6 runs) (-4.9%).
